# vwxyzjn/cleanrl

Measured on NVIDIA B200. Metric: env steps/sec (SPS) PPO Breakout num_envs=1024, higher is better.
Workload: dtype bf16

## Files before the change

### cleanrl_b200/_lib.py

```python
from __future__ import annotations

import ctypes as C
from pathlib import Path

PKG = Path(__file__).resolve().parent
LIB_PATH = PKG / "libb200rl.so"

_p = C.c_void_p
_i64 = C.c_int64
_i = C.c_int
_d = C.c_double
_sz = C.c_size_t

SIGNATURES = {
    "b200rl_version": (_i, []),
    "b200rl_last_error": (C.c_char_p, []),
    "b200rl_compiled_arch": (_i, []),
    "b200rl_launch_count": (C.c_longlong, []),
    "b200rl_profile_enable": (None, [_i]),
    "b200rl_profile_reset": (None, []),
    "b200rl_profile_summary": (_i, [C.c_char_p, _sz]),
    "b200rl_gae_f32": (_i, [_p, _p, _p, _p, _p, _p, _p, _i64, _i64, _d, _d, _i, _p]),
    "b200rl_categorical_sample_f32": (_i, [_p, _i64, _p, _p, _i64, _i64, _i, _p, _p, _p, _p, _p]),
    "b200rl_categorical_eval_f32": (_i, [_p, _i64, _p, _i64, _i, _p, _p, _p]),
    "b200rl_ppo_loss_workspace_bytes": (_sz, [_i64]),
    "b200rl_ppo_loss_f32": (_i, [_p, _i64, _p, _i64, _p, _p, _p, _p, _p, _p, _i64, _i, _d, _d, _d, _i, _i,
                                 _p, _i64, _p, _i64, _p, _p, _sz, _p]),
    "b200rl_gaussian_sample_f32": (_i, [_p, _i64, _p, _p, _p, _i64, _i64, _i, _p, _p, _p, _p, _p]),
    "b200rl_gaussian_eval_f32": (_i, [_p, _i64, _p, _p, _i64, _i, _p, _p, _p]),
    "b200rl_ppo_loss_gaussian_workspace_bytes": (_sz, [_i64]),
    "b200rl_ppo_loss_gaussian_f32": (_i, [_p, _i64, _p, _p, _i64, _p, _p, _p, _p, _p, _p, _i64, _i, _d, _d, _d, _i, _i,
                                          _p, _i64, _p, _p, _i64, _p, _p, _sz, _p]),
    "b200rl_clip_adam_workspace_bytes": (_sz, [_i64]),
    "b200rl_clip_adam_f32": (_i, [_p, _p, _p, _p, _i64, _i64, _d, _d, _d, _d, _d, _i, _p, _p, _sz, _p]),
    "b200rl_adam_step_scalars": (_i, [_i64, _d, _d, _d, _p]),
    "b200rl_clip_adam_dyn_f32": (_i, [_p, _p, _p, _p, _i64, _p, _d, _d, _d, _d, _i, _p, _p, _sz, _p]),
    "b200rl_conv2d_fwd_f32": (_i, [_p, _i, _p, _d, _p, _p, _p, _i64, _i, _i, _i, _i, _i, _i, _i, _i, _p]),
    "b200rl_conv2d_bwd_data_f32": (_i, [_p, _p, _p, _i, _p, _i64, _i, _i, _i, _i, _i, _i, _i, _p]),
    "b200rl_conv2d_bwd_weight_workspace_bytes": (_sz, [_i64, _i, _i, _i, _i, _i, _i, _i]),
    "b200rl_conv2d_bwd_weight_f32": (_i, [_p, _i, _p, _d, _p, _p, _p, _i64, _i, _i, _i, _i, _i, _i, _i, _p, _sz, _p]),
    "b200rl_conv2d_fwd_pad_f32": (_i, [_p, _i, _p, _d, _p, _p, _p, _i64, _i, _i, _i, _i, _i, _i, _i, _i, _i, _p]),
    "b200rl_conv2d_bwd_data_pad_f32": (_i, [_p, _p, _p, _i, _p, _i64, _i, _i, _i, _i, _i, _i, _i, _i, _p]),
    "b200rl_conv2d_bwd_weight_pad_workspace_bytes": (_sz, [_i64, _i, _i, _i, _i, _i, _i, _i, _i]),
    "b200rl_conv2d_bwd_weight_pad_f32": (_i, [_p, _i, _p, _d, _p, _p, _p, _i64, _i, _i, _i, _i, _i, _i, _i, _i, _p, _sz, _p]),
    "b200rl_maxpool3s2_fwd_f32": (_i, [_p, _i64, _i, _i, _p, _p, _p]),
    "b200rl_maxpool3s2_bwd_f32": (_i, [_p, _p, _i64, _i, _i, _p, _p]),
    "b200rl_relu_f32": (_i, [_p, _i64, _p, _p]),
    "b200rl_relu_bwd_f32": (_i, [_p, _p, _p, _i64, _p, _p]),
    "b200rl_add_f32": (_i, [_p, _p, _i64, _p, _p]),
    "b200rl_nhwc_to_nchw_u8": (_i, [_p, _p, _i64, _i, _i, _i, _p, _p]),
    "b200rl_linear_fwd_f32": (_i, [_p, _p, _p, _p, _p, _i64, _i, _i, _i, _p]),
    "b200rl_linear_bwd_data_f32": (_i, [_p, _p, _p, _i, _p, _i64, _i, _i, _p]),
    "b200rl_linear_bwd_weight_workspace_bytes": (_sz, [_i64, _i, _i]),
    "b200rl_linear_bwd_weight_f32": (_i, [_p, _p, _p, _p, _p, _i64, _i, _i, _p, _sz, _p]),
    "b200rl_dqn_td_loss_workspace_bytes": (_sz, [_i64]),
    "b200rl_dqn_td_loss_f32": (_i, [_p, _i64, _p, _i64, _p, _p, _p, _i64, _i, _d, _i, _p, _i64, _p, _p, _sz, _p]),
    "b200rl_argmax_f32": (_i, [_p, _i64, _i64, _i, _p, _p]),
    "b200rl_naturecnn_param_count": (_i64, [_i]),
    "b200rl_naturecnn_bf16_packed_bytes": (_sz, [_i]),
    "b200rl_naturecnn_bf16_acts_bytes": (_sz, [_i64, _i]),
    "b200rl_frames_to_s2d_bf16": (_i, [_p, _p, _i64, _p, _p]),
    "b200rl_naturecnn_bf16_workspace_bytes": (_sz, [_i64, _i]),
    "b200rl_naturecnn_bf16_pack": (_i, [_p, _i, _p, _p]),
    "b200rl_naturecnn_bf16_forward": (_i, [_p, _i, _p, _i64, _i, _p, _p, _p, _p, _p]),
    "b200rl_naturecnn_bf16_backward": (_i, [_p, _p, _i, _p, _i64, _i, _p, _p, _p, _p, _p, _p, _sz, _p, _p]),
    "b200rl_frames_to_s2d_u8": (_i, [_p, _p, _i64, _p, _p, _p]),
    "b200rl_lstm_mask_state_f32": (_i, [_p, _p, _p, _i64, _i, _p, _p, _p]),
    "b200rl_lstm_cell_fwd_f32": (_i, [_p, _p, _p, _i64, _i, _p, _p, _p, _p]),
    "b200rl_lstm_cell_bwd_f32": (_i, [_p, _p, _p, _p, _p, _p, _p, _i64, _i, _p, _p, _p]),
    "b200rl_naturecnn_grad_tail_offset": (_i64, [_i]),
    "b200rl_frames_delta_s2d_u8": (_i, [_p, _p, _p, _p, _p, _i64, _p, _p, _p]),
    "b200rl_h2d_rows_async": (_i, [_p, _p, _i64, _i64, _i64, _p]),
    "b200rl_stackdelta_create": (_p, [_i64, _i, _i64, _i]),
    "b200rl_stackdelta_destroy": (None, [_p]),
    "b200rl_stackdelta_invalidate": (None, [_p]),
    "b200rl_stackdelta_begin": (_i64, [_p, _p, _i64, _p, _p, _p, _p]),
    "b200rl_stackdelta_wait": (_i64, [_p, _p]),
    "b200rl_mt19937_shuffle_i64": (_i, [_p, _p, _p, _i64]),
    "b200rl_stackdelta_launch": (_i64, [_p, _p, _i64, _p]),
    "b200rl_stackdelta_join": (_i64, [_p, _p, _p]),
}



class PartLaunch(C.Structure):
    _fields_ = [("tracker", _p), ("copy_stream", _p), ("main_stream", _p), ("consumed_event", _p),
                ("n", C.c_int32), ("nchunks", C.c_int32), ("chunk_lo", C.c_int32 * 4), ("chunk_hi", C.c_int32 * 4),
                ("h2d_event", _p * 4), ("graph_exec", _p * 4),
                ("new_d", _p), ("slot_d", _p), ("full_d", _p), ("new_h", _p), ("full_h", _p), ("slot_h", _p),
                ("actions_d", _p), ("actions_h", _p), ("actions_bytes", _i64), ("d2h_event", _p)]


_lib = None


def load():
    global _lib
    if _lib is not None:
        return _lib
    if not LIB_PATH.exists():
        raise RuntimeError(
            f"{LIB_PATH} is missing: build it with `python -m cleanrl_b200.build` "
            "(the CUDA extension is the product; there is no CPU/torch fallback)")
    lib = C.CDLL(str(LIB_PATH))
    for name, (res, args) in SIGNATURES.items():
        fn = getattr(lib, name)
        fn.restype = res
        fn.argtypes = args
    _lib = lib
    return lib


def check(rc, what):
    if rc != 0:
        msg = load().b200rl_last_error().decode("utf-8", "replace")
        raise RuntimeError(f"libb200rl {what} failed (status {rc}): {msg}")
```

### cleanrl_b200/agents.py

```python
from __future__ import annotations

import numpy as np
import torch
import torch.nn as nn

from . import nets, ops


def layer_init(layer, std=np.sqrt(2), bias_const=0.0):
    torch.nn.init.orthogonal_(layer.weight, std)
    torch.nn.init.constant_(layer.bias, bias_const)
    return layer


def _exp_noise(n, A, device):
    return torch.empty(n, A, dtype=torch.float32, device=device).exponential_(1)


_exp_noise.graph_safe = True
_exp_noise.inplace = lambda buf: buf.exponential_(1)


class KernelAgent(nn.Module):

# ... 85 lines not shown
        return action, logprob, entropy, v.reshape(-1, 1)


class NatureCNNAgent(KernelAgent):

    def __init__(self, envs):
        super().__init__()
        c, h, w = envs.single_observation_space.shape
        assert (c, h, w) == (4, 84, 84), "NatureCNN geometry is 4x84x84"
        trunk = []
        for cin, cout, k, s in ((4, 32, 8, 4), (32, 64, 4, 2), (64, 64, 3, 1)):
            trunk += [layer_init(nn.Conv2d(cin, cout, k, stride=s)), nn.ReLU()]
        trunk += [nn.Flatten(), layer_init(nn.Linear(64 * 7 * 7, 512)), nn.ReLU()]
        self.network = nn.Sequential(*trunk)
        self.actor = layer_init(nn.Linear(512, envs.single_action_space.n), std=0.01)
        self.critic = layer_init(nn.Linear(512, 1), std=1)
        self.num_actions = int(envs.single_action_space.n)

    def _param_order(self):
        net = [p for m in self.network for p in m.parameters()]
        return net + [self.actor.weight, self.critic.weight, self.actor.bias, self.critic.bias]

    def _build_plan(self):
        f = self._flat
        A = self.num_actions
        wa, ga = f.view_of(self.actor.weight)
        ba, gba = f.view_of(self.actor.bias)
        off_w = (wa.data_ptr() - f.flat.data_ptr()) // 4
        off_b = (ba.data_ptr() - f.flat.data_ptr()) // 4
        self._head_w = f.flat[off_w:off_w + (A + 1) * 512].view(A + 1, 512)
        self._head_b = f.flat[off_b:off_b + A + 1]
        self._head_dw = f.grad[off_w:off_w + (A + 1) * 512].view(A + 1, 512)
        self._head_db = f.grad[off_b:off_b + A + 1]
        n = self.network
        self.trunk = nets.Chain([
            nets.Conv(n[0], "relu", in_div=255.0), nets.Conv(n[2], "relu"), nets.Conv(n[4], "relu"),
            nets.Linear(n[7], "relu")])
        self.head = nets.Linear(None, None, self._head_w, self._head_b, self._head_dw, self._head_db)
        self._tc = None
        self._tc_dirty = True

    precision = "fp32"

    def params_updated(self):
        self._tc_dirty = True

    def _tc_plan(self):
        f = self._flat
        if self._tc is None:
            assert f.flat.numel() >= ops._lib.load().b200rl_naturecnn_param_count(self.num_actions)
            self._tc = ops.NatureCNNBf16(self.num_actions, f.flat.device)
        if self._tc_dirty:
            self._tc.pack(f.flat)
            self._tc_dirty = False
        return self._tc

    def load_state_dict(self, *a, **k):
        out = super().load_state_dict(*a, **k)
        self._tc_dirty = True
        return out

    def pin_workspaces(self):
        if self._tc is not None:
            self._tc.pin()

    def _forward_heads(self, x, rows=None, keep=False, aux=None):
        if self.precision == "bf16":
            if x.dtype not in (torch.uint8, torch.bfloat16):
                x = x.to(torch.uint8)
            tc = self._tc_plan()
            out = tc.forward(x.contiguous(), rows, self._flat.flat)
            if keep:
                self._tc_obs, self._tc_rows, self._tc_aux = x, rows, aux
            A = self.num_actions
            return out[:, :A], out[:, A]
        if x.dtype not in (torch.uint8, torch.float32):
            x = x.float()
        hidden = self.trunk.fwd(x.contiguous(), rows=rows, keep=keep)
        out = self.head.fwd(hidden)
        if keep:
            self._hidden = hidden
        A = self.num_actions
        return out[:, :A], out[:, A]

    def forward_train(self, b_obs, mb_inds, aux=None):
        self.flat
        return self._forward_heads(b_obs, rows=mb_inds, keep=True, aux=aux)

    def alloc_head_grad(self, M, device):
        A = self.num_actions
        d = torch.empty(M, A + 1, dtype=torch.float32, device=device)
        return d, d[:, :A], d[:, A]

    def grad_tail(self):
        if self.precision != "bf16":
            return None
        if getattr(self, "_tail_event", None) is None:
            self._tail_event = torch.cuda.Event()
            self._tail_event.record()
        return self._tc_plan().grad_tail_offset(), self._tail_event

    def backward(self, dhead):
        if self.precision == "bf16":
            self._tc.backward(self._tc_obs, self._tc_rows, self._flat.flat, dhead, self._flat.grad,
                              tail_event=getattr(self, "_tail_event", None), obs_aux=getattr(self, "_tc_aux", None))
            self._tc_obs = self._tc_rows = self._tc_aux = None
            return
        hidden = self._hidden
        self.head.bwd_weight(hidden, dhead)
        dh = self.head.bwd_data(dhead, hidden, "relu")
        self.trunk.bwd(dh)
        self._hidden = None


class MLPAgent(KernelAgent):

    def __init__(self, envs):
        super().__init__()
        d = int(np.array(envs.single_observation_space.shape).prod())
        A = int(envs.single_action_space.n)
        self.critic = nn.Sequential(layer_init(nn.Linear(d, 64)), nn.Tanh(), layer_init(nn.Linear(64, 64)), nn.Tanh(),
                                    layer_init(nn.Linear(64, 1), std=1.0))
        self.actor = nn.Sequential(layer_init(nn.Linear(d, 64)), nn.Tanh(), layer_init(nn.Linear(64, 64)), nn.Tanh(),
                                   layer_init(nn.Linear(64, A), std=0.01))
        self.num_actions = A

    def _build_plan(self):
        mk = lambda seq: nets.Chain([nets.Linear(seq[0], "tanh"), nets.Linear(seq[2], "tanh"), nets.Linear(seq[4], None)])
        self.c_chain, self.a_chain = mk(self.critic), mk(self.actor)

    def _forward_heads(self, x, rows=None, keep=False):
        x = x.float() if x.dtype != torch.float32 else x
        x = x.reshape(x.shape[0], -1).contiguous()
        logits = self.a_chain.fwd(x, rows=rows, keep=keep)
        value = self.c_chain.fwd(x, rows=rows, keep=keep)
        return logits, value[:, 0]

    def forward_train(self, b_obs, mb_inds):
        self.flat
        return self._forward_heads(b_obs, rows=mb_inds, keep=True)

    def alloc_head_grad(self, M, device):
        dl = torch.empty(M, self.num_actions, dtype=torch.float32, device=device)
        dv = torch.empty(M, 1, dtype=torch.float32, device=device)
        return (dl, dv), dl, dv[:, 0]

    def backward(self, dhead):
        dl, dv = dhead
        self.a_chain.bwd(dl)
        self.c_chain.bwd(dv)


class LSTMAgent(KernelAgent):

    def __init__(self, envs):
        super().__init__()
        c, h, w = envs.single_observation_space.shape
        assert (h, w) == (84, 84), "NatureCNN trunk geometry is 84x84"
        trunk = []
        for cin, cout, k, s in ((c, 32, 8, 4), (32, 64, 4, 2), (64, 64, 3, 1)):
            trunk += [layer_init(nn.Conv2d(cin, cout, k, stride=s)), nn.ReLU()]
        trunk += [nn.Flatten(), layer_init(nn.Linear(64 * 7 * 7, 512)), nn.ReLU()]
        self.network = nn.Sequential(*trunk)
        self.lstm = nn.LSTM(512, 128)
        for name, param in self.lstm.named_parameters():
            if "bias" in name:
# ... 415 lines not shown
```

### cleanrl_b200/csrc/net_tc.cu

```cuda
#include <cuda.h>
#include "tc_base.cuh"
#include "tc_conv_win.cuh"
#include "tc_conv1_u8.cuh"
#include "tc_gemm_tma.cuh"
#include "tc_wgrad_win.cuh"
#include "tc_reduce.cuh"
#include "tc_aux.cuh"
#include "tc_heads.cuh"

namespace b200rl {

struct NatureLayout {
    int A;
    int64_t c1w, c1b, c2w, c2b, c3w, c3b, fcw, fcb, hw, hb, total;
    int64_t w1f, w2f, w2dg, w3f, w3dg, wfcf, wfcdg, w1l, w1sc, packed_total;
    explicit NatureLayout(int A_) : A(A_) {
        int64_t o = 0;
        c1w = o; o += 32 * 4 * 8 * 8;  c1b = o; o += 32;
        c2w = o; o += 64 * 32 * 4 * 4; c2b = o; o += 64;
        c3w = o; o += 64 * 64 * 3 * 3; c3b = o; o += 64;
        fcw = o; o += 512 * 3136;      fcb = o; o += 512;
        hw = o;  o += (int64_t)(A + 1) * 512;
        hb = o;  o += A + 1;
        total = o;
        int64_t q = 0;
        w1f = q; q += 32 * 256;
        w2f = q; q += 64 * 512;
        w2dg = q; q += 4 * 32 * 256;
        w3f = q; q += 64 * 576;
        w3dg = q; q += 64 * 576;
        wfcf = q; q += 512 * 3136;
        wfcdg = q; q += 3136 * 512;
        w1l = q; q += 64 * 256 / 2;
        w1sc = q; q += 64 * 2;
        packed_total = q;
    }
};

struct NatureActs {
    int64_t x0, act1, act2, act3, hid, dhid, dact3a, dact3b, dact2a, dact2b, dact1, m1, m2, m3, m4, total;
    explicit NatureActs(int64_t n, bool with_x0 = true) {
        int64_t o = 0;
        x0 = o; if (with_x0) o += n * 28224;
        act1 = o; o += n * 12800;
        act2 = o; o += n * 5184;
        act3 = o; o += n * 3136;
        hid = o;  o += n * 512;
        dhid = o; o += n * 512;
        dact3a = o; o += n * 5184;
        dact3b = o; o += n * 7744;
        dact2a = o; o += n * 6400;
        dact2b = o; o += n * 7744;
        dact1 = o; o += n * 14112;
        auto pad8 = [](int64_t v) { return (v + 7) & ~int64_t(7); };
        m1 = o; o += pad8(n * 100 * 4 * 2);
        m2 = o; o += pad8(n * 81 * 2 * 2);
        m3 = o; o += pad8(n * 49 * 2 * 2);
        m4 = o; o += pad8(n * 16 * 2);
        total = o;
    }
};

static void gemm_rowmajor(KGemmParams& p, const bf16* x, int64_t n, int nchunks) {
    memset(&p, 0, sizeof(p));
    p.scale = 1.f;
    p.A = x; p.M = n; p.nchunks = nchunks;
}


static void win_defaults(WinParams& p) { memset(&p, 0, sizeof(p)); p.scale = 1.f; }
static int round8(int v) { return (v + 7) & ~7; }
static void win_conv1(WinParams& p, const bf16* x0, const int64_t* rows, int64_t n) {
    p.A = x0; p.rows = rows; p.n = (int)n; p.G = 441; p.Wp = 21; p.M = n * 441;
    p.tpi_shift = 2;
    p.n_images = rows ? (int64_t)1 << 24 : n;
    p.ntaps = 4; p.shift[0] = 0; p.shift[1] = 1; p.shift[2] = 21; p.shift[3] = 22; p.WR = round8(128 + 22);
}
static void win_conv2(WinParams& p, const bf16* act1, int64_t n) {
    p.A = act1; p.n = (int)n; p.G = 100; p.Wp = 10; p.M = n * 100;
    p.ntaps = 4; p.shift[0] = 0; p.shift[1] = 1; p.shift[2] = 10; p.shift[3] = 11; p.WR = round8(128 + 11);
}
static void win_conv3(WinParams& p, const bf16* act2, int64_t n) {
    p.A = act2; p.n = (int)n; p.G = 81; p.Wp = 9; p.M = n * 81;
    p.ntaps = 9; for (int ky = 0; ky < 3; ++ky) for (int kx = 0; kx < 3; ++kx) p.shift[ky * 3 + kx] = ky * 9 + kx;
    p.WR = round8(128 + 20);
}
static void wgw_defaults(WGradWinParams& w) { memset(&w, 0, sizeof(w)); }

static int64_t round_up(int64_t a, int64_t b) { return ceil_div(a, b) * b; }

struct WPlan { int64_t rows_per_cta; int splits; };
// ... 88 lines not shown
    size_t b = 0;
    auto mb = [&](size_t v) { if (v > b) b = v; };
    mb(colsum_ws(n * 441, 32)); mb(colsum_ws(n * 100, 64)); mb(colsum_ws(n * 81, 64)); mb(colsum_ws(n, 512));
    mb((size_t)2 * ceil_div(n, heads_rows_per_block(n)) * (A + 1) * 514 * 4);
    return a + b + 512;
}

extern "C" int b200rl_naturecnn_bf16_pack(const float* params, int A, void* packed, void* stream) {
    B200RL_REQUIRE(params && packed && A >= 1 && A < kMaxHeads, "naturecnn_pack: bad arguments (A must be in [1,23])");
    B200RL_REQUIRE(aligned(packed, 16), "naturecnn_pack: packed buffer must be 16-B aligned");
    const NatureLayout L(A);
    bf16* P = reinterpret_cast<bf16*>(packed);
    cudaStream_t s = (cudaStream_t)stream;
    ProfScope ps(s, "pack_weights", 0, (double)L.total * 4 + (double)L.packed_total * 2);
    tc_pack_conv1_s2d<<<32, 256, 0, s>>>(params + L.c1w, P + L.w1f);
    tc_pack_conv1_i8<<<32, 256, 0, s>>>(params + L.c1w, reinterpret_cast<int8_t*>(P + L.w1l), reinterpret_cast<float*>(P + L.w1sc));
    tc_pack_conv2_cells<<<128, 256, 0, s>>>(params + L.c2w, P + L.w2f);
    tc_pack_conv_s2_classes<<<(unsigned)ceil_div(32768, 256), 256, 0, s>>>(params + L.c2w, 64, 32, P + L.w2dg);
    tc_pack_conv<<<(unsigned)ceil_div(36864, 256), 256, 0, s>>>(params + L.c3w, 64, 64, 3, 3, 0, P + L.w3f, P + L.w3dg);
    tc_pack_fc<<<dim3(512 / 8, 49 / 7), 256, 0, s>>>(params + L.fcw, 512, 49, P + L.wfcf, P + L.wfcdg);
    return check_launch("naturecnn_pack", 6);
}

extern "C" int b200rl_naturecnn_bf16_forward(const void* obs, int obs_format, const int64_t* rows, int64_t n, int A,
                                             const float* params, const void* packed, void* acts,
                                             float* head_out, void* stream) {
    B200RL_REQUIRE(n >= 0, "naturecnn_forward: negative n");
    if (n == 0) return B200RL_OK;
    B200RL_REQUIRE(obs && params && packed && acts && head_out, "naturecnn_forward: null pointer");
    B200RL_REQUIRE(A >= 1 && A < kMaxHeads, "naturecnn_forward: A=%d outside [1,23]", A);
    B200RL_REQUIRE(obs_format == B200RL_OBS_U8_NCHW || obs_format == B200RL_OBS_S2D_BF16 || obs_format == B200RL_OBS_S2D_U8,
                   "naturecnn_forward: bad obs_format %d", obs_format);
    B200RL_REQUIRE(aligned(obs, 16) && aligned(acts, 16) && aligned(packed, 16), "naturecnn_forward: misaligned buffer");
    B200RL_REQUIRE(n <= (int64_t)1 << 22, "naturecnn_forward: n too large");
    const NatureLayout L(A);
    const NatureActs Q(n, obs_format == B200RL_OBS_U8_NCHW);
    const bf16* P = reinterpret_cast<const bf16*>(packed);
    bf16* act = reinterpret_cast<bf16*>(acts);
    cudaStream_t s = (cudaStream_t)stream;
    int rc;
    KGemmParams p;
    WinParams wp;
    const bf16* x0 = reinterpret_cast<const bf16*>(obs);
    const int64_t* x0rows = rows;
    if (obs_format == B200RL_OBS_U8_NCHW) {
        if ((rc = b200rl_frames_to_s2d_bf16(reinterpret_cast<const uint8_t*>(obs), rows, n, act + Q.x0, stream))) return rc;
        x0 = act + Q.x0; x0rows = nullptr;
    }
    if (obs_format == B200RL_OBS_S2D_U8) {
        Conv1U8Params cp;
        memset(&cp, 0, sizeof(cp));
        cp.rows = rows; cp.n = (int)n; cp.n_images = rows ? (int64_t)1 << 24 : n;
        cp.limbs = reinterpret_cast<const int8_t*>(P + L.w1l); cp.sc = reinterpret_cast<const float*>(P + L.w1sc);
        cp.bias = params + L.c1b; cp.out = act + Q.act1; cp.mask_out = reinterpret_cast<uint32_t*>(act + Q.m1);
        ProfScope ps(s, "conv1_fwd", 2.0 * n * 400 * 32 * 256, (double)n * (28224 + 12800 * 2 + 1600));
        if ((rc = launch_conv1_i8(cp, obs, s, "naturecnn/conv1_i8"))) return rc;
    } else {
    win_defaults(wp); win_conv1(wp, x0, x0rows, n);
    wp.Bw = P + L.w1f; wp.N = 32; wp.vH = 20; wp.vW = 20; wp.out_mode = WOUT_S2D2; wp.out = act + Q.act1;
    wp.bias = params + L.c1b; wp.scale = 1.0f / 255.0f; wp.relu = 1; wp.mask_out = reinterpret_cast<uint32_t*>(act + Q.m1);
    { ProfScope ps(s, "conv1_fwd", 2.0 * n * 400 * 32 * 256, (double)n * ((28224 + 12800) * 2 + 1600));
      if ((rc = launch_conv_win<32, 1, 9, 4>(wp, s, "naturecnn/conv1"))) return rc; }
    }
    win_defaults(wp); win_conv2(wp, act + Q.act1, n);
    wp.Bw = P + L.w2f; wp.N = 64; wp.vH = 9; wp.vW = 9; wp.out_mode = WOUT_DENSE; wp.out = act + Q.act2;
    wp.bias = params + L.c2b; wp.relu = 1; wp.mask_out = reinterpret_cast<uint32_t*>(act + Q.m2);
    { ProfScope ps(s, "conv2_fwd", 2.0 * n * 81 * 64 * 512, (double)n * ((12800 + 5184) * 2 + 648));
      if ((rc = launch_conv_win<64, 2, 4, 4>(wp, s, "naturecnn/conv2"))) return rc; }
    win_defaults(wp); win_conv3(wp, act + Q.act2, n);
    wp.Bw = P + L.w3f; wp.N = 64; wp.vH = 7; wp.vW = 7; wp.out_mode = WOUT_DENSE; wp.out = act + Q.act3;
    wp.bias = params + L.c3b; wp.relu = 1; wp.mask_out = reinterpret_cast<uint32_t*>(act + Q.m3);
    { ProfScope ps(s, "conv3_fwd", 2.0 * n * 49 * 64 * 576, (double)n * ((5184 + 3136) * 2 + 392));
      if ((rc = launch_conv_win<64, 1, 6, 9>(wp, s, "naturecnn/conv3"))) return rc; }
    gemm_rowmajor(p, act + Q.act3, n, 49);
    p.Bw = P + L.wfcf; p.N = 512; p.out = act + Q.hid; p.ldo = 512; p.bias = params + L.fcb; p.relu = 1;
    p.mask_out = reinterpret_cast<uint32_t*>(act + Q.m4);
    { ProfScope ps(s, "fc_fwd", 2.0 * n * 512 * 3136, (double)n * (3136 + 512) * 2 + 512.0 * 3136 * 2);
      if (n <= 8192) { if ((rc = launch_gemm_tma<64, 8>(p, s, "naturecnn/fc"))) return rc; }
      else if ((rc = launch_gemm_tma<256, 4>(p, s, "naturecnn/fc"))) return rc; }
    { ProfScope ps(s, "heads_fwd", 2.0 * n * 512 * (A + 1), (double)n * (1024 + 4 * (A + 1)));
      int hb = (int)ceil_div(n, 8); if (hb > num_sms() * 8) hb = num_sms() * 8;
      tc_heads_fwd<<<hb, 256, (size_t)(A + 1) * 2048, s>>>(act + Q.hid, params + L.hw, params + L.hb, n, A + 1, 512, head_out); }
    return check_launch("naturecnn/heads");
}

extern "C" int b200rl_naturecnn_bf16_backward(const void* obs, const void* obs_aux, int obs_format, const int64_t* rows, int64_t n, int A,
                                              const float* params, const void* packed, void* acts,
                                              const float* dhead, float* grads,
                                              void* workspace, size_t workspace_bytes, void* tail_ready_event, void* stream) {
    B200RL_REQUIRE(n >= 1, "naturecnn_backward: n must be >= 1");
    B200RL_REQUIRE(obs && params && packed && acts && dhead && grads && workspace, "naturecnn_backward: null pointer");
    B200RL_REQUIRE(A >= 1 && A < kMaxHeads, "naturecnn_backward: A=%d outside [1,23]", A);
    B200RL_REQUIRE(aligned(workspace, 16), "naturecnn_backward: workspace misaligned");
    const size_t need = b200rl_naturecnn_bf16_workspace_bytes(n, A);
    if (workspace_bytes < need) return fail(B200RL_ERR_WORKSPACE, "naturecnn_backward: workspace %zu < %zu", workspace_bytes, need);
    B200RL_REQUIRE(obs_format == B200RL_OBS_U8_NCHW || obs_format == B200RL_OBS_S2D_BF16 || obs_format == B200RL_OBS_S2D_U8,
                   "naturecnn_backward: bad obs_format %d", obs_format);
    B200RL_REQUIRE(obs_format != B200RL_OBS_S2D_U8 || (obs_aux && aligned(obs_aux, 16)), "naturecnn_backward: the uint8 rollout needs obs_aux");
    const NatureLayout L(A);
    const NatureActs Q(n, obs_format == B200RL_OBS_U8_NCHW);
    const bf16* P = reinterpret_cast<const bf16*>(packed);
    bf16* act = reinterpret_cast<bf16*>(acts);
    cudaStream_t s = (cudaStream_t)stream;
    const bf16* x0 = obs_format == B200RL_OBS_U8_NCHW ? act + Q.x0 : reinterpret_cast<const bf16*>(obs);
    const int64_t* x0rows = obs_format == B200RL_OBS_U8_NCHW ? nullptr : rows;
    size_t big = 0;
    {
        auto mx = [&](size_t v) { if (v > big) big = v; };
        mx((size_t)wgrad_plan(n * 512, kC1Ctas, 128).splits * 256 * 64 * 4);
        mx((size_t)wgrad_plan(n * 100, kC2Ctas, 128).splits * 512 * 64 * 4);
        mx((size_t)wgrad_plan(n * 81, kC3Ctas, 128).splits * 640 * 64 * 4);
        mx((size_t)wgrad_plan(n, kFcSplits, 64).splits * 512 * (13 * 256) * 4);
        big = (big + 255) & ~(size_t)255;
    }
    float* wsbig = reinterpret_cast<float*>(workspace);
    float* wssmall = reinterpret_cast<float*>(reinterpret_cast<char*>(workspace) + big);
    int rc;
    const int A1 = A + 1;
    {
        const int64_t rpb = heads_rows_per_block(n);
        const int nb = (int)ceil_div(n, rpb);
        ProfScope ps(s, "heads_bwd", 4.0 * n * 512 * A1, (double)n * (2048 + 64 + 8 * A1));
        const size_t sd = (size_t)rpb * A1 * sizeof(float);
        if (A1 <= 8) tc_heads_bwd_weight<8><<<nb, 512, sd, s>>>(dhead, act + Q.hid, n, A1, 512, rpb, wssmall);
        else tc_heads_bwd_weight<kMaxHeads><<<nb, 512, sd, s>>>(dhead, act + Q.hid, n, A1, 512, rpb, wssmall);
        tc_heads_fold<<<(unsigned)ceil_div(A1 * 514, 32), 256, 0, s>>>(wssmall, 2 * nb, A1, 512, grads + L.hw, grads + L.hb);
        int db_blocks = (int)ceil_div(n * 64, 256); if (db_blocks > num_sms() * 8) db_blocks = num_sms() * 8;
        tc_heads_bwd_data<<<db_blocks, 256, (size_t)A1 * 2048, s>>>(dhead, params + L.hw, reinterpret_cast<const uint8_t*>(act + Q.m4), n, A1, 512, act + Q.dhid);
        if ((rc = check_launch("naturecnn/heads_bwd", 3))) return rc;
    }
    KGemmParams p;
    {
        const WPlan pl = wgrad_plan(n, kFcSplits, 64);
        { ProfScope ps(s, "fc_wgrad", 2.0 * n * 512 * 3136, (double)n * (3136 + 512) * 2 + 512.0 * 3136 * 4);
          CUtensorMap tmX, tmY;
          if ((rc = make_tmap_2d(&tmX, act + Q.dhid, n, 512, 64, "naturecnn/fc_wgrad"))) return rc;
          if ((rc = make_tmap_2d(&tmY, act + Q.act3, n, 3136, 64, "naturecnn/fc_wgrad"))) return rc;
          const size_t smem = (size_t)4 * (2 + 4) * 64 * 128 + 1024;
          static SmemAttrCache attr;
          if ((rc = attr.ensure(tc_wgrad_tma, smem, "naturecnn/fc_wgrad"))) return rc;
          tc_wgrad_tma<<<dim3(pl.splits, 4, 13), 160, smem, s>>>(tmX, tmY, n, pl.rows_per_cta, 2, 4, wsbig);
          if ((rc = check_launch("naturecnn/fc_wgrad"))) return rc; }
        { ProfScope ps(s, "wgrad_fold_bias", 0, 0);
          note_launches(1); tc_fold_fc<<<(unsigned)ceil_div((int64_t)512 * 3136, 256), 256, 0, s>>>(wsbig, pl.splits, 512, 13 * 256, 512, 3136, 64, 49, 1.f, grads + L.fcw);
          if ((rc = colsum(act + Q.dhid, n, 512, 512, wssmall, grads + L.fcb, s))) return rc; }
        if (tail_ready_event) {
            cudaError_t e = cudaEventRecord(reinterpret_cast<cudaEvent_t>(tail_ready_event), s);
            if (e != cudaSuccess) return fail(B200RL_ERR_CUDA, "naturecnn_backward: cudaEventRecord: %s", cudaGetErrorString(e));
        }
        gemm_rowmajor(p, act + Q.dhid, n, 8);
        p.Bw = P + L.wfcdg; p.N = 3136; p.out = act + Q.dact3a; p.out2 = act + Q.dact3b; p.dual_dact3 = 1;
        p.ldo = 3136; p.mask_bits = reinterpret_cast<const uint32_t*>(act + Q.m3);
        { ProfScope ps(s, "fc_dgrad", 2.0 * n * 512 * 3136, (double)n * ((3136 + 512) * 2 + 392) + 512.0 * 3136 * 2);
          if ((rc = launch_gemm_tma<256, 4>(p, s, "naturecnn/fc_dgrad"))) return rc; }
    }
    WGradWinParams gw;
    WinParams wp;
    FoldWin fw;
    {
        wgw_defaults(gw);
        gw.X = act + Q.act2; gw.M = n * 81; gw.n = (int)n; gw.G = 81; gw.cpr = 1; gw.nslots = 10; gw.WRX = round8(128 + 20);
        for (int t = 0; t < 9; ++t) gw.shift[t] = (t / 3) * 9 + (t % 3);
        const int st[10] = {0, 1, 2, 3, 4, 5, 6, 7, 7, 8};
        for (int k = 0; k < 10; ++k) { gw.slot_tap[k] = st[k]; gw.slot_cc[k] = 0; }
        gw.Y = act + Q.dact3a; gw.ldy = 64; gw.ncolsY = 64;
        const WPlan pl = wgrad_plan(n * 81, kC3Ctas, 128);
// ... 83 lines not shown
```

### cleanrl_b200/csrc/policy.cu

```cuda
#include "common.cuh"
#include <cfloat>

namespace b200rl {

constexpr int kMaxA = 64;

struct RowStats {
    float lse;
    float m2;
    float s2;
};

__device__ __forceinline__ RowStats row_stats(const float* __restrict__ x, int A) {
    float m = -INFINITY;
    for (int k = 0; k < A; ++k) m = fmaxf(m, x[k]);
    const float mm = (fabsf(m) == INFINITY) ? 0.f : m;
    float s = 0.f;
    for (int k = 0; k < A; ++k) s += expf(x[k] - mm);
    RowStats r;
    r.lse = logf(s) + mm;
    float m2 = -INFINITY;
    for (int k = 0; k < A; ++k) m2 = fmaxf(m2, x[k] - r.lse);
    float s2 = 0.f;
    for (int k = 0; k < A; ++k) s2 += expf((x[k] - r.lse) - m2);
    r.m2 = m2;
    r.s2 = s2;
    return r;
}

__global__ void __launch_bounds__(128) categorical_sample_kernel(
    const float* __restrict__ logits, int64_t ld, const float* __restrict__ noise,
    const float* __restrict__ value_in, int64_t ldv, int64_t n, int A,
    int64_t* __restrict__ action, float* __restrict__ logprob, float* __restrict__ entropy,
    float* __restrict__ value_out) {
    const int64_t i = (int64_t)blockIdx.x * blockDim.x + threadIdx.x;
    if (i >= n) return;
    const float* x = logits + i * ld;
    const float* q = noise + i * (int64_t)A;
    const RowStats rs = row_stats(x, A);
    float best = -INFINITY, ent = 0.f;
    int arg = 0;
    for (int k = 0; k < A; ++k) {
        const float nl = x[k] - rs.lse;
        const float p = expf(nl - rs.m2) / rs.s2;
        const float sc = p / q[k];
        if (sc > best) { best = sc; arg = k; }
        ent += fmaxf(nl, -FLT_MAX) * p;
    }
    action[i] = arg;
    logprob[i] = x[arg] - rs.lse;
    if (entropy) entropy[i] = -ent;
    if (value_out && value_in) value_out[i] = value_in[i * ldv];
}

__global__ void __launch_bounds__(128) categorical_eval_kernel(
    const float* __restrict__ logits, int64_t ld, const int64_t* __restrict__ action, int64_t n, int A,
    float* __restrict__ logprob, float* __restrict__ entropy) {
    const int64_t i = (int64_t)blockIdx.x * blockDim.x + threadIdx.x;
    if (i >= n) return;
    const float* x = logits + i * ld;
    const RowStats rs = row_stats(x, A);
    float ent = 0.f;
    for (int k = 0; k < A; ++k) {
        const float nl = x[k] - rs.lse;
        ent += fmaxf(nl, -FLT_MAX) * (expf(nl - rs.m2) / rs.s2);
    }
    int a = (int)action[i];
    a = a < 0 ? 0 : (a >= A ? A - 1 : a);
    logprob[i] = x[a] - rs.lse;
    if (entropy) entropy[i] = -ent;
}

__device__ __forceinline__ float adv_pass(const float* __restrict__ b_adv, const int64_t* __restrict__ inds, int64_t M,
                                          float mean, bool squared) {
    float s = 0.f;
    const int64_t step = blockDim.x;
    int64_t i = threadIdx.x;
    for (; i + 7 * step < M; i += 8 * step) {
        int64_t j[8];
        float v[8];
#pragma unroll
        for (int u = 0; u < 8; ++u) j[u] = inds ? __ldg(inds + i + u * step) : i + u * step;
#pragma unroll
        for (int u = 0; u < 8; ++u) v[u] = __ldg(b_adv + j[u]);
#pragma unroll
        for (int u = 0; u < 8; ++u) {
            const float d = v[u] - mean;
            s += squared ? d * d : v[u];
        }
    }
    for (; i < M; i += step) {
        const float v = b_adv[inds ? inds[i] : i];
        const float d = v - mean;
        s += squared ? d * d : v;
    }
    return s;
}
__global__ void __launch_bounds__(1024) adv_stats_kernel(
    const float* __restrict__ b_adv, const int64_t* __restrict__ inds, int64_t M, float* __restrict__ out2) {
    __shared__ float red[32];
    const float mean = block_sum(adv_pass(b_adv, inds, M, 0.f, false), red) / (float)M;
    const float ss = block_sum(adv_pass(b_adv, inds, M, mean, true), red);
    if (threadIdx.x == 0) {
        out2[0] = mean;
        out2[1] = sqrtf(ss / (float)(M - 1));
    }
}

constexpr int kLossThreads = 256;
constexpr int kNumStats = 7;

struct LossParams {
    const float* logits; int64_t ld;
    const float* value; int64_t ldv;
    const int64_t* inds;
    const int64_t* b_actions;
    const float* b_logprobs; const float* b_adv; const float* b_ret; const float* b_val;
    int64_t M; int A;
    float clip, ent_coef, vf_coef;
    int norm_adv, clip_vloss;
    float* dlogits; int64_t ldd;
    float* dvalue; int64_t lddv;
    float* stats;
    const float* adv_stats;
    float* partials;
    unsigned int* ticket;
};

__global__ void __launch_bounds__(kLossThreads) ppo_loss_kernel(LossParams P) {
    __shared__ float red[32];
    __shared__ bool is_last;
// ... 437 lines not shown
```

### cleanrl_b200/csrc/tc_base.cuh

```cuda
#pragma once
#include <cuda.h>
#include <cstring>
#include "common.cuh"
#include "tc_common.cuh"

namespace b200rl {
using namespace tc;
typedef __nv_bfloat16 bf16;

__device__ __forceinline__ int4 ldg16(const void* p) { return __ldg(reinterpret_cast<const int4*>(p)); }

typedef CUresult (*EncodeTiledFn)(CUtensorMap*, CUtensorMapDataType, cuuint32_t, void*, const cuuint64_t*, const cuuint64_t*,
                                  const cuuint32_t*, const cuuint32_t*, CUtensorMapInterleave, CUtensorMapSwizzle,
                                  CUtensorMapL2promotion, CUtensorMapFloatOOBfill);
static EncodeTiledFn g_encode = nullptr;
static int make_tmap_2d(CUtensorMap* tm, const void* base, int64_t rows, int64_t cols, int box_rows, const char* what) {
    if (!g_encode) {
        void* fn = nullptr;
        cudaDriverEntryPointQueryResult qres;
        cudaError_t e = cudaGetDriverEntryPoint("cuTensorMapEncodeTiled", &fn, cudaEnableDefault, &qres);
        if (e != cudaSuccess || qres != cudaDriverEntryPointSuccess || !fn)
            return fail(B200RL_ERR_CUDA, "%s: cuTensorMapEncodeTiled not available (%s)", what, cudaGetErrorString(e));
        g_encode = reinterpret_cast<EncodeTiledFn>(fn);
    }
    const cuuint64_t dims[2] = {(cuuint64_t)cols, (cuuint64_t)rows};
    const cuuint64_t strides[1] = {(cuuint64_t)cols * 2};
    const cuuint32_t box[2] = {64u, (cuuint32_t)box_rows};
    const cuuint32_t estr[2] = {1u, 1u};
    CUresult r = g_encode(tm, CU_TENSOR_MAP_DATA_TYPE_BFLOAT16, 2, const_cast<void*>(base), dims, strides, box, estr,
                          CU_TENSOR_MAP_INTERLEAVE_NONE, CU_TENSOR_MAP_SWIZZLE_128B, CU_TENSOR_MAP_L2_PROMOTION_L2_256B,
                          CU_TENSOR_MAP_FLOAT_OOB_FILL_NONE);
    if (r != CUDA_SUCCESS) return fail(B200RL_ERR_CUDA, "%s: cuTensorMapEncodeTiled failed (%d)", what, (int)r);
    return B200RL_OK;
}

static int make_tmap_3d(CUtensorMap* tm, const void* base, int64_t n_images, int64_t rows_per_image, int64_t cols, int box_rows,
                        const char* what) {
    if (!g_encode) {
        CUtensorMap dummy;
        int rc = make_tmap_2d(&dummy, base, 128, 64, 8, what);
        if (rc) return rc;
    }
    const cuuint64_t dims[3] = {(cuuint64_t)cols, (cuuint64_t)rows_per_image, (cuuint64_t)n_images};
    const cuuint64_t strides[2] = {(cuuint64_t)cols * 2, (cuuint64_t)rows_per_image * (cuuint64_t)cols * 2};
    const cuuint32_t box[3] = {64u, (cuuint32_t)box_rows, 1u};
    const cuuint32_t estr[3] = {1u, 1u, 1u};
    CUresult r = g_encode(tm, CU_TENSOR_MAP_DATA_TYPE_BFLOAT16, 3, const_cast<void*>(base), dims, strides, box, estr,
                          CU_TENSOR_MAP_INTERLEAVE_NONE, CU_TENSOR_MAP_SWIZZLE_128B, CU_TENSOR_MAP_L2_PROMOTION_L2_256B,
                          CU_TENSOR_MAP_FLOAT_OOB_FILL_NONE);
    if (r != CUDA_SUCCESS) return fail(B200RL_ERR_CUDA, "%s: cuTensorMapEncodeTiled (3-D) failed (%d)", what, (int)r);
    return B200RL_OK;
}

static int make_tmap_3d_u8(CUtensorMap* tm, const void* base, int64_t n_images, int64_t rows_per_image, int64_t cols, int64_t pitch,
                           int box_rows, int box_cols, const char* what) {
    if (!g_encode) {
        CUtensorMap dummy;
        int rc = make_tmap_2d(&dummy, base, 128, 64, 8, what);
        if (rc) return rc;
    }
    const cuuint64_t dims[3] = {(cuuint64_t)cols, (cuuint64_t)rows_per_image, (cuuint64_t)n_images};
    const cuuint64_t strides[2] = {(cuuint64_t)pitch, (cuuint64_t)rows_per_image * (cuuint64_t)pitch};
    const cuuint32_t box[3] = {(cuuint32_t)box_cols, (cuuint32_t)box_rows, 1u};
    const cuuint32_t estr[3] = {1u, 1u, 1u};
    CUresult r = g_encode(tm, CU_TENSOR_MAP_DATA_TYPE_UINT8, 3, const_cast<void*>(base), dims, strides, box, estr,
                          CU_TENSOR_MAP_INTERLEAVE_NONE,
                          box_cols == 64 ? CU_TENSOR_MAP_SWIZZLE_64B : (box_cols == 128 ? CU_TENSOR_MAP_SWIZZLE_128B : CU_TENSOR_MAP_SWIZZLE_NONE),
                          CU_TENSOR_MAP_L2_PROMOTION_L2_256B, CU_TENSOR_MAP_FLOAT_OOB_FILL_NONE);
    if (r != CUDA_SUCCESS) return fail(B200RL_ERR_CUDA, "%s: cuTensorMapEncodeTiled (u8 3-D) failed (%d)", what, (int)r);
    return B200RL_OK;
}

static int make_tmap_pairs_u8(CUtensorMap* tm, const void* base, int64_t n_images, const char* what) {
    if (!g_encode) {
        CUtensorMap dummy;
        int rc = make_tmap_2d(&dummy, base, 128, 64, 8, what);
        if (rc) return rc;
    }
    const cuuint64_t dims[3] = {128u, 221u, (cuuint64_t)n_images};
    const cuuint64_t strides[2] = {128u, 28224u};
    const cuuint32_t box[3] = {128u, 144u, 1u};
    const cuuint32_t estr[3] = {1u, 1u, 1u};
    CUresult r = g_encode(tm, CU_TENSOR_MAP_DATA_TYPE_UINT8, 3, const_cast<void*>(base), dims, strides, box, estr,
                          CU_TENSOR_MAP_INTERLEAVE_NONE, CU_TENSOR_MAP_SWIZZLE_128B, CU_TENSOR_MAP_L2_PROMOTION_L2_256B,
                          CU_TENSOR_MAP_FLOAT_OOB_FILL_NONE);
    if (r != CUDA_SUCCESS) return fail(B200RL_ERR_CUDA, "%s: cuTensorMapEncodeTiled (u8 pair rows) failed (%d)", what, (int)r);
    return B200RL_OK;
}

struct SmemAttrCache {
    size_t v[64] = {};
    template <class F>
    int ensure(F* func, size_t smem, const char* what) {
        int dev = 0;
        cudaGetDevice(&dev);
        const bool cached = dev >= 0 && dev < 64;
        if (cached && smem <= v[dev]) return B200RL_OK;
        cudaError_t e = cudaFuncSetAttribute(func, cudaFuncAttributeMaxDynamicSharedMemorySize, (int)smem);
        if (e != cudaSuccess) return fail(B200RL_ERR_CUDA, "%s: smem attribute (%zu B): %s", what, smem, cudaGetErrorString(e));
        if (cached) v[dev] = smem;
        return B200RL_OK;
    }
};

static int g_num_sms = 0;
static int num_sms() {
    if (g_num_sms == 0) {
        int dev = 0;
        cudaGetDevice(&dev);
        if (cudaDeviceGetAttribute(&g_num_sms, cudaDevAttrMultiProcessorCount, dev) != cudaSuccess || g_num_sms <= 0) g_num_sms = 148;
    }
    return g_num_sms;
}

}
```

### cleanrl_b200/csrc/tc_conv1_u8.cuh

```cuda
#pragma once
#include "tc_base.cuh"
#include <cuda_fp16.h>
#include <cstdlib>
#include "tc_conv_win.cuh"

namespace b200rl {
using namespace tc;

__device__ __forceinline__ void umma_i8(uint32_t tmem_d, uint64_t adesc, uint64_t bdesc, uint32_t idesc, uint32_t accumulate) {
    asm volatile(
        "{\n\t.reg .pred p;\n\t"
        "setp.ne.b32 p, %4, 0;\n\t"
        "tcgen05.mma.cta_group::1.kind::i8 [%0], %1, %2, %3, p;\n\t}\n" ::"r"(tmem_d),
        "l"(adesc), "l"(bdesc), "r"(idesc), "r"(accumulate)
        : "memory");
}
__device__ __forceinline__ void umma_f16_ts(uint32_t tmem_d, uint32_t tmem_a, uint64_t bdesc, uint32_t idesc, uint32_t accumulate) {
    asm volatile(
        "{\n\t.reg .pred p;\n\t"
        "setp.ne.b32 p, %4, 0;\n\t"
        "tcgen05.mma.cta_group::1.kind::f16 [%0], [%1], %2, %3, p;\n\t}\n" ::"r"(tmem_d),
        "r"(tmem_a), "l"(bdesc), "r"(idesc), "r"(accumulate)
        : "memory");
}
// ... 26 lines not shown
    return (uint64_t)((smem_addr & 0x3FFFFu) >> 4) | (1ull << 16) | (32ull << 32) | kDescVersion | kDescSwizzle64;
}
__device__ __forceinline__ uint32_t img64_off(int r, int c) { return (uint32_t)(r * 64 + ((c ^ ((r >> 1) & 3)) << 4)); }
__host__ __device__ constexpr uint32_t make_idesc_i8(int M, int N) {
    return (2u << 4) | (0u << 7) | (1u << 10) | ((uint32_t)(N >> 3) << 17) | ((uint32_t)(M >> 4) << 24);
}
__host__ __device__ constexpr uint32_t make_idesc_f16ts(int M, int N, int b_bf16, int b_mn_major) {
    return (1u << 4) | (0u << 7) | ((uint32_t)b_bf16 << 10) | ((uint32_t)b_mn_major << 16) | ((uint32_t)(N >> 3) << 17) |
           ((uint32_t)(M >> 4) << 24);
}

__global__ void __launch_bounds__(256) tc_frames_to_s2d_u8(const uint8_t* __restrict__ obs, const int64_t* __restrict__ rows, int64_t n,
                                                           uint8_t* __restrict__ out_rm, uint8_t* __restrict__ out_cm) {
    __shared__ __align__(16) uint8_t plane[7056];
    const int64_t i = blockIdx.x >> 2;
    const int c = blockIdx.x & 3;
    const int64_t img = rows ? rows[i] : i;
    const int4* src = reinterpret_cast<const int4*>(obs + img * 28224 + c * 7056);
    for (int t = threadIdx.x; t < 441; t += 256) reinterpret_cast<int4*>(plane)[t] = __ldg(src + t);
    __syncthreads();
    for (int pos = threadIdx.x; pos < 441; pos += 256) {
        const int Y = pos / 21, X = pos - Y * 21;
        const uint8_t* p = plane + (Y * 4) * 84 + X * 4;
        int4 v;
        v.x = *reinterpret_cast<const int*>(p); v.y = *reinterpret_cast<const int*>(p + 84);
        v.z = *reinterpret_cast<const int*>(p + 168); v.w = *reinterpret_cast<const int*>(p + 252);
        *reinterpret_cast<int4*>(out_rm + (i * 441 + pos) * 64 + c * 16) = v;
    }
    for (int t = threadIdx.x; t < 16 * 112; t += 256) {
        const int ch = t / 112, q = t - ch * 112;
        const int sy = ch >> 2, sx = ch & 3;
        uint32_t w = 0;
#pragma unroll
        for (int e = 0; e < 4; ++e) {
            const int pos = q * 4 + e;
            if (pos < 441) {
                const int Y = pos / 21, X = pos - Y * 21;
                w |= (uint32_t)plane[(Y * 4 + sy) * 84 + X * 4 + sx] << (8 * e);
            }
        }
        *reinterpret_cast<uint32_t*>(out_cm + (i * 64 + c * 16 + ch) * 448 + q * 4) = w;
    }
}

__global__ void __launch_bounds__(256) tc_pack_conv1_i8(const float* __restrict__ w, int8_t* __restrict__ limbs, float* __restrict__ sc) {
    __shared__ float red[32];
    const int co = blockIdx.x, idx = threadIdx.x;
    const float v = w[co * 256 + idx];
    float m = fabsf(v);
#pragma unroll
    for (int o = 16; o > 0; o >>= 1) m = fmaxf(m, __shfl_xor_sync(0xffffffffu, m, o));
    if ((idx & 31) == 0) red[idx >> 5] = m;
    __syncthreads();
    float mx = red[0];
#pragma unroll
    for (int k = 1; k < 8; ++k) mx = fmaxf(mx, red[k]);
    const float s = mx > 0.f ? mx * (128.0f / 127.0f) : 1.0f;
    const float u = v / s * 128.0f;
    float l1 = rintf(u);
    l1 = fminf(fmaxf(l1, -127.f), 127.f);
    float l2 = rintf((u - l1) * 128.0f);
    l2 = fminf(fmaxf(l2, -127.f), 127.f);
    const int kx = idx & 7, ky = (idx >> 3) & 7, c = idx >> 6;
    const int a = ky >> 2, sy = ky & 3, b = kx >> 2, sx = kx & 3;
    const int k = (a * 2 + b) * 64 + c * 16 + sy * 4 + sx;
    limbs[co * 256 + k] = (int8_t)l1;
    limbs[(32 + co) * 256 + k] = (int8_t)l2;
    if (idx == 0) {
        sc[co] = s / 128.0f / 255.0f;
        sc[32 + co] = s / 16384.0f / 255.0f;
    }
}

struct Conv1U8Params {
    const int64_t* rows;
    int n;
    int64_t n_images;
    const int8_t* limbs;
    const float* sc;
    const float* bias;
    bf16* out;
    uint32_t* mask_out;
};

constexpr bool kConv1I8Direct256 = true;
template <int STAGES, int DBG>
__global__ void __launch_bounds__(kConvWinThreads, 1) tc_conv1_i8(const __grid_constant__ CUtensorMap tmA, const Conv1U8Params p, int total_tiles) {
    constexpr int BN = 64, WR = 144, NTAPS = 4;
    constexpr int STAGE_BYTES = WR * 128;
    constexpr int B_CHUNK = BN * 64;
    constexpr int NT = 4;
    constexpr uint32_t TMEM_COLS = 2 * NT * BN;
    extern __shared__ uint8_t smem_raw[];
    __shared__ uint64_t full_bar[STAGES], empty_bar[STAGES], tfull_bar[2 * NT], tempty_bar[2 * NT];
    __shared__ uint32_t tmem_base_smem;
    __shared__ __align__(16) float s_sc[32], s_bias[32];
    uint8_t* smem = reinterpret_cast<uint8_t*>((reinterpret_cast<uintptr_t>(smem_raw) + 1023) & ~uintptr_t(1023));
    const int tid = threadIdx.x, warp = tid >> 5;
    uint8_t* sW = smem;
    uint8_t* sRing = smem + NTAPS * B_CHUNK;
    uint8_t* sStage = sRing + (size_t)STAGES * STAGE_BYTES;

    if (tid == 0) {
        for (int s = 0; s < STAGES; ++s) { mbar_init(&full_bar[s], 1); mbar_init(&empty_bar[s], 1); }
        for (int a = 0; a < 2 * NT; ++a) { mbar_init(&tfull_bar[a], 1); mbar_init(&tempty_bar[a], 4); }
        fence_barrier_init();
        tma_prefetch_desc(&tmA);
    }
    if (warp == 1) tmem_alloc(&tmem_base_smem, TMEM_COLS);
    for (int idx = tid; idx < NTAPS * BN * 4; idx += blockDim.x) {
        const int c16 = idx & 3;
        const int t = (idx >> 2) & 3;
        const int r = idx >> 4;
        *reinterpret_cast<int4*>(sW + t * B_CHUNK + img64_off(r, c16)) = ldg16(p.limbs + r * 256 + t * 64 + c16 * 16);
    }
    if (tid < 32) { s_sc[tid] = p.sc[32 + tid]; s_bias[tid] = p.bias[tid]; }
    fence_proxy_async_smem();
    tc_fence_before_sync();
    __syncthreads();
    tc_fence_after_sync();
    const uint32_t tmem_d = tmem_base_smem;
    const int tile_begin = (int)(((int64_t)total_tiles * blockIdx.x) / gridDim.x);
    const int tile_end = (int)(((int64_t)total_tiles * (blockIdx.x + 1)) / gridDim.x);

    if (warp == 0) {
        if (tid == 0) {
            uint32_t q = 0;
            int z_next = 0;
            if (tile_begin < tile_end) {
                const int img = tile_begin >> 1;
                z_next = p.rows ? (int)__ldg(p.rows + img) : img;
            }
            for (int tile = tile_begin; tile < tile_end; ++tile, ++q) {
                const uint32_t s = q % STAGES;
                const int z = z_next;
                if (tile + 1 < tile_end) {
                    const int img = (tile + 1) >> 1;
                    z_next = p.rows ? (int)__ldg(p.rows + img) : img;
                }
                if (q >= (uint32_t)STAGES) mbar_wait(&empty_bar[s], ((q / STAGES) - 1) & 1);
                if (DBG & 2) { mbar_arrive(&full_bar[s]); continue; }
                mbar_arrive_expect_tx(&full_bar[s], (uint32_t)STAGE_BYTES);
                tma_load_3d(smem_u32(sRing + (size_t)s * STAGE_BYTES), &tmA, 0, (tile & 1) * 128, z, &full_bar[s]);
            }
        }
    } else if (warp == 1) {
        const bool leader = elect_one();
        constexpr uint32_t idesc = make_idesc_i8(128, BN);
        const uint64_t a_hi = desc_kmajor(0) & 0xFFFFFFFF00000000ull;
        const uint32_t a_flags = (uint32_t)(desc_kmajor(0) & 0xFFFFFFFFull);
        const uint64_t b_hi = desc_kmajor_sw64(0) & 0xFFFFFFFF00000000ull;
        const uint32_t b_flags = (uint32_t)(desc_kmajor_sw64(0) & 0xFFFFFFFFull);
        const uint32_t w_lo = ((smem_u32(sW) & 0x3FFFFu) >> 4) | b_flags;
        constexpr int off[4] = {0, 1, 21, 22};
        uint32_t q = 0;
        for (int tile = tile_begin; tile < tile_end; ++tile, ++q) {
            const uint32_t s = q % STAGES;
            mbar_wait(&full_bar[s], (q / STAGES) & 1);
            const uint32_t win_lo = ((smem_u32(sRing + (size_t)s * STAGE_BYTES) & 0x3FFFFu) >> 4) | a_flags;
#pragma unroll
            for (int e = 0; e < 2; ++e) {
                const uint32_t acc = 2 * (q % NT) + e;
                if (q >= (uint32_t)NT) mbar_wait(&tempty_bar[acc], ((q / NT) - 1) & 1);
                tc_fence_after_sync();
                if (leader) {
                    const uint32_t d_addr = tmem_d + acc * BN;
#pragma unroll
                    for (int t = 0; t < NTAPS; ++t) {
                        if (DBG & 4) break;
                        const int po = e + off[t];
                        const uint32_t a_lo = win_lo + (uint32_t)((po >> 1) * 8 + (po & 1) * 4);
                        const uint32_t b_lo = w_lo + (uint32_t)((t * B_CHUNK) >> 4);
#pragma unroll
                        for (int kk = 0; kk < 2; ++kk)
                            umma_i8(d_addr, a_hi | (uint64_t)(a_lo + 2 * kk), b_hi | (uint64_t)(b_lo + 2 * kk), idesc,
                                    (t | kk) != 0 ? 1u : 0u);
                    }
                    if (e == 1) umma_commit(&empty_bar[s]);
                    umma_commit(&tfull_bar[acc]);
                }
                __syncwarp();
            }
        }
    } else {
        const int ew = warp & 3;
        const int grp = (warp - 2) >> 2;
        const int e = grp & 1, tp = grp >> 1;
        const int lrow = ew * 32 + (tid & 31);
        const uint32_t lane_base = tmem_d + ((uint32_t)(ew * 32) << 16);
        for (int tile = tile_begin + tp; tile < tile_end; tile += 2) {
            const uint32_t k = (uint32_t)(tile - tile_begin);
            const uint32_t acc = 2 * (k % NT) + e;
            const uint32_t lane_addr = lane_base + acc * BN;
            const int i = tile >> 1;
            const int rem = 2 * (((tile & 1) << 7) + lrow) + e;
            const int Y = (rem * 3121) >> 16, X = rem - Y * 21;
            const bool valid = rem < 441 && Y < 20 && X < 20;
            const int64_t cell = ((int64_t)i * 10 + (Y >> 1)) * 10 + (X >> 1);
            const int cls = (Y & 1) * 2 + (X & 1);
            mbar_wait(&tfull_bar[acc], (k / NT) & 1);
            tc_fence_after_sync();
            uint32_t a1[32], a2[32];
            if (DBG & 8) {
#pragma unroll
                for (int c4 = 0; c4 < 32; ++c4) { a1[c4] = (uint32_t)(tile + c4); a2[c4] = (uint32_t)(lrow * c4); }
            } else {
                tmem_ld32(lane_addr, a1);
                tmem_ld32(lane_addr + 32, a2);
                tmem_ld_wait();
            }
            tc_fence_before_sync();
            __syncwarp();
            if ((tid & 31) == 0) mbar_arrive(&tempty_bar[acc]);
            uint32_t bits = 0u;
            uint32_t pk[16];
#pragma unroll
            for (int c4 = 0; c4 < 32; c4 += 4) {
                const float4 sc = *reinterpret_cast<const float4*>(s_sc + c4);
                const float4 bi = *reinterpret_cast<const float4*>(s_bias + c4);
                const float f0 = fmaf((float)((int)a1[c4] * 128 + (int)a2[c4]), sc.x, bi.x);
                const float f1 = fmaf((float)((int)a1[c4 + 1] * 128 + (int)a2[c4 + 1]), sc.y, bi.y);
                const float f2 = fmaf((float)((int)a1[c4 + 2] * 128 + (int)a2[c4 + 2]), sc.z, bi.z);
                const float f3 = fmaf((float)((int)a1[c4 + 3] * 128 + (int)a2[c4 + 3]), sc.w, bi.w);
                bits |= (f0 > 0.f ? 1u : 0u) << c4;
                bits |= (f1 > 0.f ? 1u : 0u) << (c4 + 1);
                bits |= (f2 > 0.f ? 1u : 0u) << (c4 + 2);
                bits |= (f3 > 0.f ? 1u : 0u) << (c4 + 3);
                pk[c4 >> 1] = pack_bf16x2_relu(f0, f1);
                pk[(c4 >> 1) + 1] = pack_bf16x2_relu(f2, f3);
            }
            if (valid && !(DBG & 1)) p.mask_out[cell * 4 + cls] = bits;
            if (kConv1I8Direct256) {
                if (valid && !(DBG & 1)) {
                    uint8_t* dst = reinterpret_cast<uint8_t*>(p.out) + (cell * 4 + cls) * 64;
                    st_global_256(dst, make_int4((int)pk[0], (int)pk[1], (int)pk[2], (int)pk[3]), make_int4((int)pk[4], (int)pk[5], (int)pk[6], (int)pk[7]));
                    st_global_256(dst + 32, make_int4((int)pk[8], (int)pk[9], (int)pk[10], (int)pk[11]),
                                  make_int4((int)pk[12], (int)pk[13], (int)pk[14], (int)pk[15]));
                }
                continue;
            }
            uint8_t* stg = sStage + (size_t)(warp - 2) * 2304;
            const int lane = tid & 31;
            {
                const uint32_t f = (uint32_t)(lane >> 1) & 3u;
#pragma unroll
                for (int c = 0; c < 4; ++c)
                    *reinterpret_cast<int4*>(stg + lane * 64 + ((((uint32_t)c) ^ f) << 4)) =
                        make_int4((int)pk[4 * c], (int)pk[4 * c + 1], (int)pk[4 * c + 2], (int)pk[4 * c + 3]);
                reinterpret_cast<int*>(stg + 2048)[lane] = valid ? (int)(cell * 4 + cls) : -1;
            }
            __syncwarp();
#pragma unroll
            for (int i2 = 0; i2 < 4; ++i2) {
                const int R = (lane >> 2) + 8 * i2, c = lane & 3;
                const int unit = reinterpret_cast<const int*>(stg + 2048)[R];
                const int4 v = *reinterpret_cast<const int4*>(stg + R * 64 + ((((uint32_t)c) ^ ((uint32_t)(R >> 1) & 3u)) << 4));
                if (unit >= 0 && !(DBG & 1)) *reinterpret_cast<int4*>(reinterpret_cast<uint8_t*>(p.out) + (int64_t)unit * 64 + c * 16) = v;
            }
            __syncwarp();
        }
    }
    tc_fence_before_sync();
    __syncthreads();
    if (warp == 1) tmem_dealloc(tmem_d, TMEM_COLS);
}

struct Conv1WgradU8Params {
    const int64_t* rows;
    int n;
    int64_t rows_per_cta;
    float* ws;
    float* wsb;
};
constexpr int kC1WXStages = 12, kC1WYStages = 14;
constexpr int kC1WBlock = 64 * 128, kC1WYBytes = 128 * 64, kC1WYPadRows = 24, kC1WYPad = kC1WYPadRows * 64;
constexpr int kC1WShift = 21;
constexpr float kDact1Scale = 4096.0f;

__device__ __forceinline__ uint32_t prmt(uint32_t a, uint32_t b, uint32_t sel) {
    uint32_t d;
    asm("prmt.b32 %0, %1, %2, %3;" : "=r"(d) : "r"(a), "r"(b), "r"(sel));
    return d;
}
template <int B, int NH>
__device__ __forceinline__ void u8_to_f16_biased(const uint32_t* W, uint32_t (&H)[NH]) {
#pragma unroll
    for (int j = 0; j < NH / 2; ++j) {
        uint32_t x = W[j];
        if (B == 1) x = prmt(W[j], W[j + 1], 0x4321u);
        if (B == 2) x = prmt(W[j], W[j + 1], 0x5432u);
        if (B == 3) x = prmt(W[j], W[j + 1], 0x6543u);
        H[2 * j] = prmt(x, 0x64646464u, 0x5140u);
        H[2 * j + 1] = prmt(x, 0x64646464u, 0x7362u);
    }
}
constexpr float kU8Bias = 1024.0f;

constexpr int kC1WConvWarps = 16;
constexpr int kC1WThreads = (4 + kC1WConvWarps + 4 + 2) * 32;
template <int DBG>
__global__ void __launch_bounds__(kC1WThreads, 1) tc_conv1_wgrad_u8(const __grid_constant__ CUtensorMap tmX, const __grid_constant__ CUtensorMap tmY,
                                                                  const __grid_constant__ CUtensorMap tmYpad, const Conv1WgradU8Params p) {
    constexpr int XS = kC1WXStages, YS = kC1WYStages;
    constexpr int NA = 6;
    constexpr uint32_t TMEM_COLS = 512, COL_D = 0, COL_A = 128;
    extern __shared__ uint8_t smem_raw[];
    __shared__ uint64_t xfull[XS], xempty[XS], yfull[YS], yempty[YS], a_full[NA], a_empty[NA], done_bar;
    __shared__ uint32_t tmem_base_smem;
    __shared__ float sRed[32 * 32], sBias[32];
    uint8_t* smem = reinterpret_cast<uint8_t*>((reinterpret_cast<uintptr_t>(smem_raw) + 1023) & ~uintptr_t(1023));
    uint8_t* sX = smem;
    uint8_t* sYpad = smem + (size_t)XS * kC1WBlock;
    uint8_t* sYb = sYpad + kC1WYPad;
// ... 267 lines not shown
```

### cleanrl_b200/csrc/tc_conv_win.cuh

```cuda
#pragma once
#include "tc_base.cuh"

namespace b200rl {
using namespace tc;

enum { WOUT_DENSE = 0, WOUT_S2D2 = 1, WOUT_DACT2 = 2, WOUT_DACT1 = 3 };
struct WinParams {
    const bf16* A;
    const int64_t* rows;
    int64_t M;
    int n, G, Wp;
    int tpi_shift;
    int64_t n_images;
    int ntaps;
    int shift[16];
    int WR;
    const bf16* Bw;
    int N;
    int vH, vW;
    int out_mode;
    bf16* out;
    bf16* out2;
    const uint32_t* mask_bits;
    uint32_t* mask_out;
    const float* bias;
    float scale;
    int relu;
    int out_f16;
};

__device__ __forceinline__ uint32_t pack_f16x2_sat(float lo, float hi) {
    uint32_t d;
    asm("cvt.rn.satfinite.f16x2.f32 %0, %1, %2;" : "=r"(d) : "f"(hi), "f"(lo));
    return d;
}

constexpr int kConvWinThreads = 576;
__host__ __device__ constexpr int conv_win_groups(int BN) { return BN >= 128 ? 2 : 4; }
__host__ __device__ constexpr int conv_win_threads(int BN) { return 64 + conv_win_groups(BN) * 128; }
__host__ __device__ constexpr int conv_win_acc_bufs(int BN) { return BN <= 128 ? 4 : 2; }
template <int BN, int CPR, int STAGES, int NTAPS>
__global__ void __launch_bounds__(conv_win_threads(BN), 1) tc_conv_win(const __grid_constant__ CUtensorMap tmA, const WinParams p,
                                                      int total_tiles) {
    constexpr int B_CHUNK = BN * 128;
    constexpr int NB = conv_win_acc_bufs(BN);
    constexpr int NG = conv_win_groups(BN);
    static_assert(NB % NG == 0, "every epilogue group owns NB / NG accumulator buffers");
    constexpr uint32_t TMEM_COLS = (NB * BN) < 32 ? 32 : NB * BN;
    extern __shared__ uint8_t smem_raw[];
    __shared__ uint64_t full_bar[STAGES], empty_bar[STAGES], tfull_bar[NB], tempty_bar[NB];
    __shared__ uint32_t tmem_base_smem;
    uint8_t* smem = reinterpret_cast<uint8_t*>((reinterpret_cast<uintptr_t>(smem_raw) + 1023) & ~uintptr_t(1023));
    const int tid = threadIdx.x, warp = tid >> 5;
    const int nchunks = p.ntaps * CPR;
    const int K = nchunks * 64;
    const int IMG = p.WR * 128;
    const int STAGE_BYTES = IMG * CPR;
    uint8_t* sW = smem;
    uint8_t* sRing = smem + (size_t)nchunks * B_CHUNK;

    if (tid == 0) {
        for (int s = 0; s < STAGES; ++s) { mbar_init(&full_bar[s], 1); mbar_init(&empty_bar[s], 1); }
        for (int a = 0; a < NB; ++a) { mbar_init(&tfull_bar[a], 1); mbar_init(&tempty_bar[a], 4); }
        fence_barrier_init();
        tma_prefetch_desc(&tmA);
    }
    if (warp == 1) tmem_alloc(&tmem_base_smem, TMEM_COLS);
    for (int idx = tid; idx < nchunks * BN * 8; idx += blockDim.x) {
        const int c16 = idx & 7;
        int t = idx >> 3;
        const int r = t % BN; const int j = t / BN;
        int4 v = make_int4(0, 0, 0, 0);
        if (r < p.N) v = ldg16(p.Bw + (int64_t)r * K + j * 64 + c16 * 8);
        *reinterpret_cast<int4*>(sW + (size_t)j * B_CHUNK + img_off(r, c16)) = v;
    }
    fence_proxy_async_smem();
    tc_fence_before_sync();
    __syncthreads();
    tc_fence_after_sync();
    const uint32_t tmem_d = tmem_base_smem;
    const int tile_begin = (int)(((int64_t)total_tiles * blockIdx.x) / gridDim.x);
    const int tile_end = (int)(((int64_t)total_tiles * (blockIdx.x + 1)) / gridDim.x);

    if (warp == 0) {
        if (tid == 0) {
            uint32_t q = 0;
            const int tmask = (1 << p.tpi_shift) - 1;
            int z_next = 0;
            if (p.tpi_shift && tile_begin < tile_end) {
                const int img = tile_begin >> p.tpi_shift;
                z_next = p.rows ? (int)__ldg(p.rows + img) : img;
            }
            for (int tile = tile_begin; tile < tile_end; ++tile, ++q) {
                const uint32_t s = q % STAGES;
                const int z = z_next;
                if (p.tpi_shift && tile + 1 < tile_end) {
                    const int img = (tile + 1) >> p.tpi_shift;
                    z_next = p.rows ? (int)__ldg(p.rows + img) : img;
                }
                if (q >= (uint32_t)STAGES) mbar_wait(&empty_bar[s], ((q / STAGES) - 1) & 1);
                const uint32_t dst = smem_u32(sRing + (size_t)s * STAGE_BYTES);
                mbar_arrive_expect_tx(&full_bar[s], (uint32_t)STAGE_BYTES);
                if (p.tpi_shift) {
#pragma unroll
                    for (int c = 0; c < CPR; ++c) tma_load_3d(dst + c * IMG, &tmA, c * 64, (tile & tmask) * 128, z, &full_bar[s]);
                } else {
#pragma unroll
                    for (int c = 0; c < CPR; ++c) tma_load_2d(dst + c * IMG, &tmA, c * 64, tile * 128, &full_bar[s]);
                }
            }
        }
    } else if (warp == 1) {
        const bool leader = elect_one();
        constexpr uint32_t idesc = make_idesc(128, BN, 0, 0);
        const uint64_t desc_hi = desc_kmajor(0) & 0xFFFFFFFF00000000ull;
        const uint32_t desc_lo_flags = (uint32_t)(desc_kmajor(0) & 0xFFFFFFFFull);
        const uint32_t w_lo = ((smem_u32(sW) & 0x3FFFFu) >> 4) | desc_lo_flags;
// ... 11 lines not shown
                    for (int c = 0; c < CPR; ++c) {
                        const uint32_t a_lo = win_lo + (uint32_t)((c * IMG) >> 4) + (uint32_t)p.shift[t] * 8u;
                        const uint32_t b_lo = w_lo + (uint32_t)(((t * CPR + c) * B_CHUNK) >> 4);
#pragma unroll
                        for (int kk = 0; kk < 4; ++kk)
                            umma_bf16(d_addr, desc_hi | (uint64_t)(a_lo + 2 * kk), desc_hi | (uint64_t)(b_lo + 2 * kk), idesc,
                                      (t | c | kk) != 0 ? 1u : 0u);
                    }
                }
                umma_commit(&empty_bar[s]);
                umma_commit(&tfull_bar[acc]);
            }
            __syncwarp();
        }
    } else {
        const int ew = warp & 3;
        const int h = (warp - 2) >> 2;
        const int lrow = ew * 32 + (tid & 31);
        const uint32_t mW = (65536u + (uint32_t)p.Wp - 1u) / (uint32_t)p.Wp;
        constexpr int TSTEP = NG * 128;
        const int step_i = TSTEP / p.G, step_rem = TSTEP % p.G;
        int64_t r = ((int64_t)tile_begin + h) * 128 + lrow;
        int i_lin = (int)(r / p.G);
        int rem_lin = (int)(r - (int64_t)i_lin * p.G);
        const int tmask = (1 << p.tpi_shift) - 1;
        const uint32_t lane_base = tmem_d + ((uint32_t)(ew * 32) << 16);
        constexpr int NW = BN / 32;
        uint32_t k = 0;
        for (int tile = tile_begin + h; tile < tile_end; tile += NG, ++k) {
            const uint32_t acc = (uint32_t)(tile - tile_begin) % NB;
            const uint32_t lane_addr = lane_base + acc * BN;
            int i = i_lin, rem = rem_lin;
            bool inside = r < p.M;
            if (p.tpi_shift) {
                i = tile >> p.tpi_shift;
                rem = ((tile & tmask) << 7) + lrow;
                inside = rem < p.G;
            }
            const int Y = (int)(((uint32_t)rem * mW) >> 16), X = rem - Y * p.Wp;
            const bool valid = inside && (Y < p.vH) && (X < p.vW);
            int64_t o1 = 0, o2 = 0, ob = 0;
            if (p.out_mode == WOUT_DENSE) {
                const int64_t orow = ((int64_t)i * p.vH + Y) * p.vW + X;
                o1 = orow * p.N; ob = orow * (p.N >> 5);
            } else if (p.out_mode == WOUT_S2D2) {
                const int64_t cell = ((int64_t)i * 10 + (Y >> 1)) * 10 + (X >> 1);
                const int cls = (Y & 1) * 2 + (X & 1);
                o1 = cell * 128 + cls * 32; ob = cell * 4 + cls;
            } else if (p.out_mode == WOUT_DACT2) {
                o1 = ((int64_t)i * 100 + Y * 10 + X) * 64;
                o2 = ((int64_t)i * 121 + (Y + 1) * 11 + (X + 1)) * 64;
                ob = ((int64_t)i * 81 + Y * 9 + X) * 2;
            } else {
                ob = ((int64_t)i * 100 + Y * 10 + X) * 4;
            }
            uint32_t mb[NW];
#pragma unroll
            for (int g = 0; g < NW; ++g) mb[g] = 0xFFFFFFFFu;
            if (p.mask_bits != nullptr && valid) {
                if (NW == 4) {
                    const int4 t = ldg16(p.mask_bits + ob);
                    mb[0] = (uint32_t)t.x; mb[1 % NW] = (uint32_t)t.y; mb[2 % NW] = (uint32_t)t.z; mb[3 % NW] = (uint32_t)t.w;
                } else if (NW == 2) {
                    const uint2 t = __ldg(reinterpret_cast<const uint2*>(p.mask_bits + ob));
                    mb[0] = t.x; mb[1 % NW] = t.y;
                } else {
                    mb[0] = __ldg(p.mask_bits + ob);
                }
            }
            mbar_wait(&tfull_bar[acc], ((uint32_t)(tile - tile_begin) / NB) & 1);
            tc_fence_after_sync();
#pragma unroll
            for (int g = 0; g < NW; ++g) {
                uint32_t v[32];
                tmem_ld32(lane_addr + g * 32, v);
                tmem_ld_wait();
                if (g == NW - 1) {
                    tc_fence_before_sync();
                    __syncwarp();
                    if ((tid & 31) == 0) mbar_arrive(&tempty_bar[acc]);
                }
                if (!valid || g * 32 >= p.N) continue;
                if (p.bias) {
                    const float4* bp = reinterpret_cast<const float4*>(p.bias + g * 32);
#pragma unroll
                    for (int e = 0; e < 8; ++e) {
                        const float4 bv = __ldg(bp + e);
                        v[4 * e] = __float_as_uint(fmaf(__uint_as_float(v[4 * e]), p.scale, bv.x));
                        v[4 * e + 1] = __float_as_uint(fmaf(__uint_as_float(v[4 * e + 1]), p.scale, bv.y));
                        v[4 * e + 2] = __float_as_uint(fmaf(__uint_as_float(v[4 * e + 2]), p.scale, bv.z));
                        v[4 * e + 3] = __float_as_uint(fmaf(__uint_as_float(v[4 * e + 3]), p.scale, bv.w));
                    }
                } else {
#pragma unroll
                    for (int e = 0; e < 32; ++e) v[e] = __float_as_uint(__uint_as_float(v[e]) * p.scale);
                }
                if (p.relu) {
                    uint32_t bits = 0u;
#pragma unroll
                    for (int e = 0; e < 32; ++e) {
                        const float f = __uint_as_float(v[e]);
                        bits |= (f > 0.f ? 1u : 0u) << e;
                    }
                    if (p.mask_out) p.mask_out[ob + g] = bits;
                }
                if (p.mask_bits) {
#pragma unroll
                    for (int e = 0; e < 32; ++e) if (!((mb[g] >> e) & 1u)) v[e] = 0u;
                }
                int4 w[4];
                if (p.out_f16) {
#pragma unroll
                    for (int e = 0; e < 4; ++e) {
                        w[e].x = (int)pack_f16x2_sat(__uint_as_float(v[8 * e]), __uint_as_float(v[8 * e + 1]));
                        w[e].y = (int)pack_f16x2_sat(__uint_as_float(v[8 * e + 2]), __uint_as_float(v[8 * e + 3]));
                        w[e].z = (int)pack_f16x2_sat(__uint_as_float(v[8 * e + 4]), __uint_as_float(v[8 * e + 5]));
                        w[e].w = (int)pack_f16x2_sat(__uint_as_float(v[8 * e + 6]), __uint_as_float(v[8 * e + 7]));
                    }
                } else if (p.relu) {
#pragma unroll
                    for (int e = 0; e < 4; ++e) {
                        w[e].x = (int)pack_bf16x2_relu(__uint_as_float(v[8 * e]), __uint_as_float(v[8 * e + 1]));
                        w[e].y = (int)pack_bf16x2_relu(__uint_as_float(v[8 * e + 2]), __uint_as_float(v[8 * e + 3]));
                        w[e].z = (int)pack_bf16x2_relu(__uint_as_float(v[8 * e + 4]), __uint_as_float(v[8 * e + 5]));
                        w[e].w = (int)pack_bf16x2_relu(__uint_as_float(v[8 * e + 6]), __uint_as_float(v[8 * e + 7]));
                    }
                } else {
#pragma unroll
                for (int e = 0; e < 4; ++e) {
                    w[e].x = (int)pack_bf16x2(__uint_as_float(v[8 * e]), __uint_as_float(v[8 * e + 1]));
                    w[e].y = (int)pack_bf16x2(__uint_as_float(v[8 * e + 2]), __uint_as_float(v[8 * e + 3]));
                    w[e].z = (int)pack_bf16x2(__uint_as_float(v[8 * e + 4]), __uint_as_float(v[8 * e + 5]));
                    w[e].w = (int)pack_bf16x2(__uint_as_float(v[8 * e + 6]), __uint_as_float(v[8 * e + 7]));
                }
                }
                bf16* dst;
                if (p.out_mode == WOUT_DACT1) {
                    dst = p.out + ((int64_t)i * 441 + (2 * Y + (g >> 1)) * 21 + 2 * X + (g & 1)) * 32;
                } else {
                    dst = p.out + o1 + g * 32;
                }
                st_global_256(dst, w[0], w[1]);
                st_global_256(dst + 16, w[2], w[3]);
                if (p.out_mode == WOUT_DACT2) {
                    bf16* dst2 = p.out2 + o2 + g * 32;
                    st_global_256(dst2, w[0], w[1]);
                    st_global_256(dst2 + 16, w[2], w[3]);
                }
            }
            r += TSTEP; i_lin += step_i; rem_lin += step_rem;
            if (rem_lin >= p.G) { rem_lin -= p.G; ++i_lin; }
        }
    }
    tc_fence_before_sync();
    __syncthreads();
    if (warp == 1) tmem_dealloc(tmem_d, TMEM_COLS);
}

template <int BN, int CPR, int STAGES, int NTAPS>
static int launch_conv_win(const WinParams& p, cudaStream_t s, const char* what) {
    if (p.ntaps != NTAPS) return fail(B200RL_ERR_INVALID_ARGUMENT, "%s: %d taps, kernel instance has %d", what, p.ntaps, NTAPS);
    const size_t smem = (size_t)p.ntaps * CPR * BN * 128 + (size_t)STAGES * p.WR * 128 * CPR + 1024;
    static SmemAttrCache attr;
    if (int rc = attr.ensure(tc_conv_win<BN, CPR, STAGES, NTAPS>, smem, what)) return rc;
    if ((int64_t)p.G * p.Wp >= 65536 || p.G < 1 || p.N % 32 != 0)
        return fail(B200RL_ERR_INVALID_ARGUMENT, "%s: grid %d x width %d outside the epilogue's multiply-shift range, or N %% 32 != 0", what, p.G, p.Wp);
    if (p.rows && !p.tpi_shift) return fail(B200RL_ERR_INVALID_ARGUMENT, "%s: the image gather needs image-aligned tiling", what);
    if (p.tpi_shift && (128 << p.tpi_shift) < p.G) return fail(B200RL_ERR_INVALID_ARGUMENT, "%s: tiles per image too small", what);
    const int total = p.tpi_shift ? (int)((int64_t)p.n << p.tpi_shift) : (int)ceil_div(p.M, 128);
    int grid = num_sms();
    if (grid > total) grid = total;
    CUtensorMap tmA;
    memset(&tmA, 0, sizeof(tmA));
    int rc;
    if (p.tpi_shift) rc = make_tmap_3d(&tmA, p.A, p.n_images, p.G, (int64_t)CPR * 64, p.WR, what);
    else rc = make_tmap_2d(&tmA, p.A, p.M, (int64_t)CPR * 64, p.WR, what);
    if (rc) return rc;
    tc_conv_win<BN, CPR, STAGES, NTAPS><<<grid, conv_win_threads(BN), smem, s>>>(tmA, p, total);
    return check_launch(what);
}

}
```

### cleanrl_b200/csrc/tc_heads.cuh

```cuda
#pragma once
#include "tc_base.cuh"
#include "tc_reduce.cuh"

namespace b200rl {
using namespace tc;

constexpr int kMaxHeads = 24;
constexpr int kHeadsPartialBlocks = 296;
static inline int64_t heads_rows_per_block(int64_t n) {
    int64_t rpb = (n + kHeadsPartialBlocks - 1) / kHeadsPartialBlocks;
    if (rpb < 16) rpb = 16;
    if (rpb > 256) rpb = 256;
    return rpb;
}

__global__ void __launch_bounds__(256) tc_heads_fwd(const bf16* __restrict__ hid, const float* __restrict__ Wh,
                                                    const float* __restrict__ bh, int64_t n, int A1, int H,
                                                    float* __restrict__ out) {
    extern __shared__ float sW[];
    for (int i = threadIdx.x; i < A1 * 512; i += blockDim.x) sW[i] = Wh[i];
    __syncthreads();
    const int lane = threadIdx.x & 31, wpb = blockDim.x >> 5;
    for (int64_t row = (int64_t)blockIdx.x * wpb + (threadIdx.x >> 5); row < n; row += (int64_t)gridDim.x * wpb) {
        float hv[16];
        const bf16* hp = hid + row * 512;
#pragma unroll
        for (int q = 0; q < 2; ++q) {
            const int4 v = ldg16(hp + q * 256 + lane * 8);
            const uint32_t w[4] = {(uint32_t)v.x, (uint32_t)v.y, (uint32_t)v.z, (uint32_t)v.w};
#pragma unroll
            for (int e = 0; e < 4; ++e) {
                hv[q * 8 + 2 * e] = __uint_as_float(w[e] << 16);
                hv[q * 8 + 2 * e + 1] = __uint_as_float(w[e] & 0xFFFF0000u);
            }
        }
        float mine = 0.f;
        for (int a = 0; a < A1; ++a) {
            float s = 0.f;
#pragma unroll
            for (int q = 0; q < 2; ++q) {
                const float4 w0 = *reinterpret_cast<const float4*>(sW + a * 512 + q * 256 + lane * 8);
                const float4 w1 = *reinterpret_cast<const float4*>(sW + a * 512 + q * 256 + lane * 8 + 4);
                s = fmaf(hv[q * 8 + 0], w0.x, s); s = fmaf(hv[q * 8 + 1], w0.y, s);
                s = fmaf(hv[q * 8 + 2], w0.z, s); s = fmaf(hv[q * 8 + 3], w0.w, s);
                s = fmaf(hv[q * 8 + 4], w1.x, s); s = fmaf(hv[q * 8 + 5], w1.y, s);
                s = fmaf(hv[q * 8 + 6], w1.z, s); s = fmaf(hv[q * 8 + 7], w1.w, s);
            }
            s = warp_sum(s);
            if (lane == a) mine = s + bh[a];
        }
        if (lane < A1) out[row * A1 + lane] = mine;
    }
}
__global__ void __launch_bounds__(256) tc_heads_bwd_data(const float* __restrict__ dhead, const float* __restrict__ Wh,
                                                         const uint8_t* __restrict__ hid_bits, int64_t n, int A1, int H,
                                                         bf16* __restrict__ dhid) {
    extern __shared__ float sWt[];
    for (int i = threadIdx.x; i < A1 * 512; i += blockDim.x) {
        const int a = i >> 9, h = i & 511;
        sWt[a * 512 + (h & 7) * 64 + (h >> 3)] = Wh[i];
    }
    __syncthreads();
    const int64_t total = n * 64;
    for (int64_t idx = (int64_t)blockIdx.x * blockDim.x + threadIdx.x; idx < total; idx += (int64_t)gridDim.x * blockDim.x) {
        const int64_t row = idx >> 6;
        const int g = (int)(idx & 63);
        const uint32_t m = hid_bits[idx];
        float o[8];
#pragma unroll
        for (int e = 0; e < 8; ++e) o[e] = 0.f;
        for (int a = 0; a < A1; ++a) {
            const float d = __ldg(dhead + row * A1 + a);
#pragma unroll
            for (int e = 0; e < 8; ++e) o[e] = fmaf(d, sWt[a * 512 + e * 64 + g], o[e]);
        }
#pragma unroll
        for (int e = 0; e < 8; ++e) if (!((m >> e) & 1u)) o[e] = 0.f;
        int4 w;
        w.x = (int)pack_bf16x2(o[0], o[1]); w.y = (int)pack_bf16x2(o[2], o[3]);
        w.z = (int)pack_bf16x2(o[4], o[5]); w.w = (int)pack_bf16x2(o[6], o[7]);
        *reinterpret_cast<int4*>(dhid + row * 512 + g * 8) = w;
    }
}
template <int MAXA>
__global__ void __launch_bounds__(512) tc_heads_bwd_weight(const float* __restrict__ dhead, const bf16* __restrict__ hid,
                                                           int64_t n, int A1, int H, int64_t rows_per_block,
                                                           float* __restrict__ part) {
    extern __shared__ float sD[];
    const int hp = threadIdx.x & 255, rl = threadIdx.x >> 8;
    const int64_t r0 = (int64_t)blockIdx.x * rows_per_block;
    int64_t r1 = r0 + rows_per_block;
    if (r1 > n) r1 = n;
    const int nrows = (int)(r1 > r0 ? r1 - r0 : 0);
    for (int i = threadIdx.x; i < nrows * A1; i += blockDim.x) sD[i] = dhead[r0 * A1 + i];
    __syncthreads();
    float acc0[MAXA], acc1[MAXA], bacc[MAXA];
#pragma unroll
    for (int a = 0; a < MAXA; ++a) { acc0[a] = 0.f; acc1[a] = 0.f; bacc[a] = 0.f; }
    const uint32_t* h2 = reinterpret_cast<const uint32_t*>(hid);
    int r = rl;
    for (; r + 14 < nrows; r += 16) {
        uint32_t hv[8];
#pragma unroll
        for (int u = 0; u < 8; ++u) hv[u] = __ldg(h2 + (r0 + r + 2 * u) * 256 + hp);
#pragma unroll
        for (int u = 0; u < 8; ++u) {
            const float x0 = __uint_as_float(hv[u] << 16), x1 = __uint_as_float(hv[u] & 0xFFFF0000u);
            const float* dr = sD + (r + 2 * u) * A1;
#pragma unroll
            for (int a = 0; a < MAXA; ++a) {
                if (a < A1) {
                    const float d = dr[a];
                    acc0[a] = fmaf(d, x0, acc0[a]); acc1[a] = fmaf(d, x1, acc1[a]); bacc[a] += d;
                }
            }
        }
    }
    for (; r < nrows; r += 2) {
        const uint32_t hv = __ldg(h2 + (r0 + r) * 256 + hp);
        const float x0 = __uint_as_float(hv << 16), x1 = __uint_as_float(hv & 0xFFFF0000u);
        const float* dr = sD + r * A1;
#pragma unroll
        for (int a = 0; a < MAXA; ++a) {
            if (a < A1) {
                const float d = dr[a];
                acc0[a] = fmaf(d, x0, acc0[a]); acc1[a] = fmaf(d, x1, acc1[a]); bacc[a] += d;
            }
        }
    }
    float* pb = part + ((int64_t)blockIdx.x * 2 + rl) * A1 * (H + 2);
#pragma unroll
    for (int a = 0; a < MAXA; ++a) {
        if (a < A1) {
            *reinterpret_cast<float2*>(pb + (int64_t)a * (H + 2) + 2 * hp) = make_float2(acc0[a], acc1[a]);
// ... 17 lines not shown
```

### cleanrl_b200/ops.py

```python
from __future__ import annotations

import torch

from . import _lib

STAT_NAMES = ("pg_loss", "v_loss", "entropy", "old_approx_kl", "approx_kl", "clipfrac", "loss",
              "adv_mean", "adv_std")


def _stream():
    return torch.cuda.current_stream().cuda_stream


def _ptr(t, dtype=None, name="tensor", allow_none=False):
    if t is None:
        if allow_none:
            return None
        raise ValueError(f"{name} is None")
    if not isinstance(t, torch.Tensor) or not t.is_cuda:
        raise RuntimeError(f"{name}: libb200rl kernels need a CUDA tensor (got {type(t).__name__} on "
                           f"{getattr(t, 'device', '?')}); there is no CPU fallback")
    if dtype is not None and t.dtype != dtype:
        raise TypeError(f"{name}: expected {dtype}, got {t.dtype}")
    return t.data_ptr()
# ... 361 lines not shown
    lib = _lib.load()
    n, H = c_masked.shape
    f = torch.float32
    for nm, t in (("gates_x", gates_x), ("gates_h", gates_h), ("c_masked", c_masked), ("h_out", h_out), ("c_out", c_out)):
        _contig(t, nm)
    assert gates_x.shape == (n, 4 * H) and gates_h.shape == (n, 4 * H)
    rc = lib.b200rl_lstm_cell_fwd_f32(_ptr(gates_x, f, "gates_x"), _ptr(gates_h, f, "gates_h"), _ptr(c_masked, f, "c_masked"), n, H,
                                      _ptr(h_out, f, "h_out"), _ptr(c_out, f, "c_out"), _ptr(save, f, "save", True), _stream())
    _lib.check(rc, "lstm_cell_fwd")


def lstm_cell_bwd(dh_heads, dh_rec_raw, done_next, dc_rec, save, c_masked, done, dgates, dc_rec_out):
    lib = _lib.load()
    n, H = c_masked.shape
    f = torch.float32
    for nm, t in (("dh_heads", dh_heads), ("save", save), ("c_masked", c_masked), ("done", done), ("dgates", dgates),
                  ("dc_rec_out", dc_rec_out)):
        _contig(t, nm)
    rc = lib.b200rl_lstm_cell_bwd_f32(_ptr(dh_heads, f, "dh_heads"), _ptr(dh_rec_raw, f, "dh_rec_raw", True),
                                      _ptr(done_next, f, "done_next", True), _ptr(dc_rec, f, "dc_rec", True), _ptr(save, f, "save"),
                                      _ptr(c_masked, f, "c_masked"), _ptr(done, f, "done"), n, H, _ptr(dgates, f, "dgates"),
                                      _ptr(dc_rec_out, f, "dc_rec_out"), _stream())
    _lib.check(rc, "lstm_cell_bwd")


class NatureCNNBf16:

    def __init__(self, A, device):
        lib = _lib.load()
        self.A, self.device = int(A), device
        self.param_count = lib.b200rl_naturecnn_param_count(self.A)
        self.packed = torch.empty(lib.b200rl_naturecnn_bf16_packed_bytes(self.A), dtype=torch.uint8, device=device)
        self._acts = {}
        self._pinned = set()
        self._ws = None

    MAX_UNPINNED = 4

    def pin(self):
        self._pinned.update(self._acts.keys())

    def acts(self, n, fmt):
        lib = _lib.load()
        key = (n, fmt)
        buf = self._acts.pop(key, None)
        if buf is None:
            unpinned = [k for k in self._acts if k not in self._pinned]
            while len(unpinned) >= self.MAX_UNPINNED:
                del self._acts[unpinned.pop(0)]
            buf = torch.zeros(lib.b200rl_naturecnn_bf16_acts_bytes(n, fmt), dtype=torch.uint8, device=self.device)
        self._acts[key] = buf
        return buf

    @staticmethod
    def obs_format(obs):
        if obs.dtype == torch.uint8 and obs.dim() >= 4 and tuple(obs.shape[-3:]) == (4, 84, 84):
            return 0
        if obs.dtype == torch.bfloat16 and tuple(obs.shape[-3:]) == (21, 21, 64):
            return 1
        if obs.dtype == torch.uint8 and tuple(obs.shape[-2:]) == (441, 64):
            return 2
        raise TypeError("tensor-core NatureCNN path consumes uint8 [*,4,84,84] frames, uint8 space-to-depth rollout rows "
                        f"[*,441,64] or space-to-depth bf16 [*,21,21,64] (got {obs.dtype} {tuple(obs.shape)})")

    def pack(self, flat_params):
        lib = _lib.load()
        rc = lib.b200rl_naturecnn_bf16_pack(_ptr(flat_params, torch.float32, "params"), self.A,
                                            self.packed.data_ptr(), _stream())
        _lib.check(rc, "naturecnn_bf16_pack")

    def forward(self, obs, rows, flat_params, head_out=None):
        lib = _lib.load()
        fmt = self.obs_format(obs)
        _contig(obs, "obs")
        n = rows.numel() if rows is not None else obs.shape[0]
        if head_out is None:
            head_out = torch.empty(n, self.A + 1, dtype=torch.float32, device=self.device)
        rc = lib.b200rl_naturecnn_bf16_forward(_ptr(obs, None, "obs"), fmt, _ptr(rows, torch.int64, "rows", True), n, self.A,
                                               _ptr(flat_params, torch.float32, "params"), self.packed.data_ptr(),
                                               self.acts(n, fmt).data_ptr(), _ptr(head_out, torch.float32, "head_out"), _stream())
        _lib.check(rc, "naturecnn_bf16_forward")
        return head_out

    def grad_tail_offset(self):
        return int(_lib.load().b200rl_naturecnn_grad_tail_offset(self.A))

    def backward(self, obs, rows, flat_params, dhead, flat_grads, tail_event=None, obs_aux=None):
        lib = _lib.load()
        fmt = self.obs_format(obs)
        if fmt == 2:
            if obs_aux is None or obs_aux.dtype != torch.uint8 or tuple(obs_aux.shape[-2:]) != (64, 448) or \
                    obs_aux.shape[0] != obs.shape[0]:
                raise ValueError("uint8 rollout rows need their channel-major copy [*,64,448] (obs_aux) for the backward pass")
            _contig(obs_aux, "obs_aux")
        n = dhead.shape[0]
        _contig(dhead, "dhead")
        nbytes = lib.b200rl_naturecnn_bf16_workspace_bytes(n, self.A)
        if self._ws is None or self._ws.numel() < nbytes:
            self._ws = torch.empty(nbytes, dtype=torch.uint8, device=self.device)
        rc = lib.b200rl_naturecnn_bf16_backward(_ptr(obs, None, "obs"), _ptr(obs_aux, None, "obs_aux", True), fmt,
                                                _ptr(rows, torch.int64, "rows", True), n, self.A,
                                                _ptr(flat_params, torch.float32, "params"), self.packed.data_ptr(),
                                                self.acts(n, fmt).data_ptr(), _ptr(dhead, torch.float32, "dhead"),
                                                _ptr(flat_grads, torch.float32, "grads"),
                                                self._ws.data_ptr(), self._ws.numel(),
                                                tail_event.cuda_event if tail_event is not None else None, _stream())
        _lib.check(rc, "naturecnn_bf16_backward")


def frames_to_s2d(obs_u8, out=None, rows=None):
    lib = _lib.load()
    _contig(obs_u8, "obs")
    n = rows.numel() if rows is not None else obs_u8.shape[0]
    if out is None:
        out = torch.empty(n, 21, 21, 64, dtype=torch.bfloat16, device=obs_u8.device)
    rc = lib.b200rl_frames_to_s2d_bf16(_ptr(obs_u8, torch.uint8, "obs"), _ptr(rows, torch.int64, "rows", True), n,
                                       _ptr(out, torch.bfloat16, "out"), _stream())
    _lib.check(rc, "frames_to_s2d")
    return out


def alloc_u8_rollout_rows(shape, device):
    n = 1
    for d in shape:
        n *= int(d)
    flat = torch.zeros(n + 256, dtype=torch.uint8, device=device)
    return flat[:n].view(*shape)


def frames_to_s2d_u8(obs_u8, out_rm=None, out_cm=None, rows=None):
    lib = _lib.load()
    _contig(obs_u8, "obs")
    n = rows.numel() if rows is not None else obs_u8.shape[0]
    if out_rm is None:
        out_rm = alloc_u8_rollout_rows((n, 441, 64), obs_u8.device)
    if out_cm is None:
        out_cm = torch.empty(n, 64, 448, dtype=torch.uint8, device=obs_u8.device)
    _contig(out_rm, "out_rm"); _contig(out_cm, "out_cm")
    assert out_rm.shape[0] == n and out_cm.shape[0] == n
    rc = lib.b200rl_frames_to_s2d_u8(_ptr(obs_u8, torch.uint8, "obs"), _ptr(rows, torch.int64, "rows", True), n,
                                     _ptr(out_rm, torch.uint8, "out_rm"), _ptr(out_cm, torch.uint8, "out_cm"), _stream())
    _lib.check(rc, "frames_to_s2d_u8")
    return out_rm, out_cm


def frames_delta_s2d_u8(new_planes, prev_rm, prev_cm, out_rm, out_cm, full_slot=None, full_frames=None):
    lib = _lib.load()
    n = new_planes.shape[0]
    for nm, t in (("new_planes", new_planes), ("prev_rm", prev_rm), ("prev_cm", prev_cm), ("out_rm", out_rm), ("out_cm", out_cm)):
        _contig(t, nm)
        assert t.shape[0] == n, nm
    if full_slot is not None:
        _contig(full_slot, "full_slot"); _contig(full_frames, "full_frames")
        assert full_slot.shape[0] == n
    rc = lib.b200rl_frames_delta_s2d_u8(_ptr(new_planes, torch.uint8, "new_planes"), _ptr(full_slot, torch.int32, "full_slot", True),
                                        _ptr(full_frames, torch.uint8, "full_frames", True), _ptr(prev_rm, torch.uint8, "prev_rm"),
                                        _ptr(prev_cm, torch.uint8, "prev_cm"), n, _ptr(out_rm, torch.uint8, "out_rm"),
                                        _ptr(out_cm, torch.uint8, "out_cm"), _stream())
    _lib.check(rc, "frames_delta_s2d_u8")


def h2d_rows_async(dst, src_ptr, src_pitch, row_bytes, rows, stream=None):
    lib = _lib.load()
    assert dst.is_contiguous() and dst.numel() * dst.element_size() >= rows * row_bytes
    rc = lib.b200rl_h2d_rows_async(dst.data_ptr(), src_ptr, src_pitch, row_bytes, rows,
                                   stream.cuda_stream if stream is not None else _stream())
# ... 165 lines not shown
```

### cleanrl_b200/ppo_engine.py

```python
from __future__ import annotations

import os
import time

import numpy as np
import torch

from . import ops

STAT_NAMES = ops.STAT_NAMES


def _torch_dtype(np_dtype):
    return torch.uint8 if np.dtype(np_dtype) == np.uint8 else torch.float32


def _pin(t):
    return t.pin_memory() if torch.cuda.is_available() else t


def _sync():
    if torch.cuda.is_available():
        torch.cuda.current_stream().synchronize()

# ... 50 lines not shown
        self.next_done = torch.zeros(N, dtype=f32, device=device)
        self.next_value = torch.zeros(N, dtype=f32, device=device)
        self.rewards_h = _pin(torch.zeros((T, N), dtype=f32))
        self.dones_h = _pin(torch.zeros((T, N), dtype=f32))
        self.next_done_h = _pin(torch.zeros(N, dtype=f32))
        self.actions_h = _pin(torch.zeros_like(self.actions[0], device="cpu"))
        self.obs_stage_h = _pin(torch.zeros((N,) + tuple(obs_shape), dtype=self.obs_dtype))
        E = int(args.update_epochs)
        self.b_inds_h = _pin(torch.zeros((E, self.B), dtype=torch.int64))
        self.b_inds = torch.zeros((E, self.B), dtype=torch.int64, device=device)
        n_upd = int(args.update_epochs) * self.num_minibatches
        self.stats = torch.zeros(max(n_upd, 1), 16, dtype=f32, device=device)
        self.stats_h = _pin(torch.zeros(max(n_upd, 1), 16, dtype=f32))
        self.grad_norm = torch.zeros(1, dtype=f32, device=device)
        self.update_graphs = os.environ.get("CLEANRL_B200_UPDATE_GRAPHS", "1") != "0"
        self.host_seconds = {"shuffle": 0.0, "update_enqueue": 0.0, "update_wait": 0.0}
        self._shuffle = (ops.numpy_global_shuffle if device.type == "cuda" and os.environ.get("CLEANRL_B200_NATIVE_SHUFFLE", "1") != "0"
                         else np.random.shuffle)
        self._upd_graphs, self._upd_kernels, self._upd_iters = {}, {}, 0
        self.hyper = torch.zeros(max(n_upd, 1), 2, dtype=f32, device=device)
        self.hyper_h = _pin(torch.zeros(max(n_upd, 1), 2, dtype=f32))
        self.flat = agent.flat
        if self.overlap_exchange and hasattr(agent, "grad_tail"):
            agent.grad_tail()
        if cuda_graphs is None:
            cuda_graphs = os.environ.get("CLEANRL_B200_CUDA_GRAPHS", "1") != "0"
        self.cuda_graphs = bool(cuda_graphs) and device.type == "cuda"
        chunks = int(os.environ.get("CLEANRL_B200_H2D_CHUNKS", "4"))
        self.h2d_chunks = chunks if (self.cuda_graphs and getattr(self, "s2d", False) and chunks > 1
                                     and N % chunks == 0 and N // chunks >= 128) else 1
        C = self.h2d_chunks
        if C == 4 and N % 16 == 0:
            sizes = [5 * N // 16, 5 * N // 16, 4 * N // 16, 2 * N // 16]
        else:
            sizes = [N // C] * C
        self.chunk_bounds = [(sum(sizes[:c]), sum(sizes[:c + 1])) for c in range(C)]
        self.noise_buf = None
        if self.h2d_chunks > 1:
            self.copy_stream = torch.cuda.Stream(device=device)
            self.chunk_events = [torch.cuda.Event() for _ in range(self.h2d_chunks)]
            self.noise_buf = torch.zeros(agent.noise_shape(N), dtype=f32, device=device)
        self._parts = None
        want_delta = os.environ.get("CLEANRL_B200_DELTA_UPLOAD")
        if want_delta is None:
            want_delta = "1" if int(os.environ.get("LOCAL_WORLD_SIZE", "1") or 1) <= 1 else "0"
        self.delta_upload = bool(getattr(self, "u8_rollout", False)) and want_delta != "0"
        self._delta_allowed = self.delta_upload
        self._delta = None
        self.delta_redos = 0
        self.delta_full_frames = 0
        self._graphs = {}
        self._graph_pool = None
        self._graph_kernels = {}
        self._graph_warm = set()
        self.graph_launches = 0
        self.h2d_bytes = 0
        self.d2h_bytes = 0
        self.kernel_launches = 0

    def _to_storage(self, src_u8, step, sl=slice(None)):
        dst = self.next_obs if step is None else self.obs[step]
        if self.u8_rollout:
            dst_t = self.next_obs_t if step is None else self.obs_t[step]
            ops.frames_to_s2d_u8(src_u8, dst[sl], dst_t[sl])
        else:
            ops.frames_to_s2d(src_u8, out=dst[sl])

    def _upload_obs(self, step, obs_np, convert=True):
        dst = self.next_obs if step is None else self.obs[step]
        src = torch.from_numpy(np.ascontiguousarray(obs_np))
        if src.dtype != self.obs_dtype:
            src = src.to(self.obs_dtype)
        if not src.is_pinned():
            self.obs_stage_h.copy_(src)
            src = self.obs_stage_h
        if self.s2d:
            self.obs_u8.copy_(src, non_blocking=True)
            if convert:
                self._to_storage(self.obs_u8, step)
        else:
            dst.copy_(src, non_blocking=True)
        self.h2d_bytes += src.numel() * src.element_size()

    def _step_device_work(self, step, noise=None):
        if self.s2d:
            self._to_storage(self.obs_u8, step)
        self.agent.sample_into(self.obs[step], self.actions[step], self.logprobs[step], self.values[step], noise=noise)

    def _chunk_device_work(self, step, c):
        sl = slice(*self.chunk_bounds[c])
        self._to_storage(self.obs_u8[sl], step, sl)
        self.agent.sample_into(self.obs[step][sl], self.actions[step][sl], self.logprobs[step][sl],
                               self.values[step][sl], noise=self.noise_buf[sl])

    def _run_step(self, step, chunk=None):
        if chunk is not None:
            work, key = (lambda: self._chunk_device_work(step, chunk)), (step, chunk)
            return self._run_graphed(work, key, warm_key=("c", chunk))
        if self._graphable() and not getattr(self.agent.noise_fn, "graph_safe", False):
            if self.noise_buf is None:
                self.noise_buf = torch.zeros(self.agent.noise_shape(self.N), dtype=torch.float32, device=self.device)
            self.agent.draw_noise_into(self.noise_buf)
            return self._run_graphed(lambda: self._step_device_work(step, noise=self.noise_buf), step, warm_key=("f", 0))
        return self._run_graphed(lambda: self._step_device_work(step), step, warm_key=("f", 0))

    def _graphable(self):
        return self.cuda_graphs and getattr(self.agent, "graph_capturable", getattr(self.agent, "graph_friendly", False))

    def _run_graphed(self, work, key, warm_key):
        if not self._graphable():
            return work()
        if hasattr(self.agent, "_tc_plan") and getattr(self.agent, "precision", "fp32") == "bf16":
            self.agent._tc_plan()
        g = self._graphs.get(key)
        if g is None:
            if warm_key not in self._graph_warm:
                rng = torch.cuda.get_rng_state(self.device)
                work()
                torch.cuda.current_stream().synchronize()
                torch.cuda.set_rng_state(rng, self.device)
                self._graph_warm.add(warm_key)
            from . import _lib
            l0 = _lib.load().b200rl_launch_count()
            g = torch.cuda.CUDAGraph()
            if self._graph_pool is None:
                self._graph_pool = torch.cuda.graph_pool_handle()
            with torch.cuda.graph(g, pool=self._graph_pool):
                work()
            self._graphs[key] = g
            if hasattr(self.agent, "pin_workspaces"):
                self.agent.pin_workspaces()
            self._graph_kernels[key] = _lib.load().b200rl_launch_count() - l0
        g.replay()
        self.graph_launches += self._graph_kernels[key]

    @torch.no_grad()
    def policy_step(self, step, next_obs_np, next_done_np):
        if self.h2d_chunks > 1 and self._graphable():
            self._pipelined_step(step, next_obs_np)
            self.dones_h[step].copy_(torch.as_tensor(np.asarray(next_done_np, dtype=np.float32)))
        else:
            self.dones_h[step].copy_(torch.as_tensor(np.asarray(next_done_np, dtype=np.float32)))
            self._upload_obs(step, next_obs_np, convert=False)
            self._run_step(step)
        self.actions_h.copy_(self.actions[step], non_blocking=True)
        self.d2h_bytes += self.actions_h.numel() * self.actions_h.element_size()
        _sync()
        return self.actions_h.numpy()

    def _pipelined_step(self, step, obs_np):
        src = torch.from_numpy(np.ascontiguousarray(obs_np))
        if not src.is_pinned():
            self.obs_stage_h.copy_(src)
            src = self.obs_stage_h
        C = self.h2d_chunks
        main = torch.cuda.current_stream()
        with torch.cuda.stream(self.copy_stream):
            for c, (lo, hi) in enumerate(self.chunk_bounds):
                self.obs_u8[lo:hi].copy_(src[lo:hi], non_blocking=True)
                self.chunk_events[c].record(self.copy_stream)
        self.h2d_bytes += src.numel()
        self.agent.draw_noise_into(self.noise_buf)
        for c in range(C):
            main.wait_event(self.chunk_events[c])
            self._run_step(step, chunk=c)

    @torch.no_grad()
    def policy_step_resident(self, step, obs_dev, done_dev=None):
        if self.s2d and obs_dev.dtype == torch.uint8:
            self.obs_u8.copy_(obs_dev)
        else:
            self.obs[step].copy_(obs_dev)
        self._run_step(step)

    @torch.no_grad()
    def rollout_resident(self, obs_pool):
        P = obs_pool.shape[0]

        def work():
            for step in range(self.T):
                src = obs_pool[step % P]
                if self.s2d and src.dtype == torch.uint8:
                    self._to_storage(src, step)
                else:
                    self.obs[step].copy_(src)
                self.agent.sample_into(self.obs[step], self.actions[step], self.logprobs[step], self.values[step])

        if not getattr(self.agent, "graph_friendly", False):
            return work()
        self._run_graphed(work, ("rollout", obs_pool.data_ptr(), P), warm_key="r")

    def _part_setup(self, P):
        if getattr(self, "_parts", None) is not None and len(self._parts) == P:
            return
        N = self.N
        assert N % P == 0, "num_envs must be divisible by the number of env groups"
        n = N // P
        self._parts = [(p * n, (p + 1) * n) for p in range(P)]
        C = 2 if (n % 2 == 0 and n // 2 >= 64 and self.s2d and self._graphable()) else 1
        want = os.environ.get("CLEANRL_B200_PART_CHUNKS")
        if want and self.s2d and self._graphable() and 1 <= int(want) <= 4 and n % int(want) == 0:
            C = int(want)
        self._part_chunks = [[(lo + c * (n // C), lo + (c + 1) * (n // C)) for c in range(C)] for lo, hi in self._parts]
        if getattr(self, "copy_stream", None) is None:
            self.copy_stream = torch.cuda.Stream(device=self.device)
        self._part_h2d = [[torch.cuda.Event() for _ in ch] for ch in self._part_chunks]
        self._part_d2h = [torch.cuda.Event() for _ in range(P)]
        if self.noise_buf is None:
            self.noise_buf = torch.zeros(self.agent.noise_shape(N), dtype=torch.float32, device=self.device)
        if not hasattr(self, "obs_u8"):
            self.obs_u8 = None
        self._noise_bufs = [self.noise_buf, torch.zeros_like(self.noise_buf)]
        self._noise_step = -1
        self._actions_np = self.actions_h.numpy()
        self._rewards_np, self._dones_np = self.rewards_h.numpy(), self.dones_h.numpy()
        self._dones_ptr = self.dones_h.data_ptr()
        self._part_d2h_bytes = n * self.actions_h.element_size() * max(1, self.act_dim)
        self._part_d2h_handles = [None] * P
        self._plans, self._plan_refs, self._plan_kernels, self._plan_stream = {}, {}, {}, None
        if self.device.type == "cuda":
            from . import _lib
            self._lib = _lib.load()
        self._delta = None
        if self._delta_allowed and self._graphable():
            u8 = torch.uint8
            self._delta = [dict(tr=ops.StackDeltaTracker(n), full_d=torch.zeros((n, 28224), dtype=u8, device=self.device),
                                last=None, boot_obs=None, consumed=torch.cuda.Event()) for _ in range(P)]
            self._new_d = torch.zeros((N, 7056), dtype=u8, device=self.device)
            self._slot_d = torch.zeros(N, dtype=torch.int32, device=self.device)
            self._mis_ptr = [d["tr"].mis_h.data_ptr() for d in self._delta]

    def _part_work(self, step, lo, hi):
        sl = slice(lo, hi)
        if self.s2d:
            self._to_storage(self.obs_u8[sl], step, sl)
        self.agent.sample_into(self.obs[step][sl], self.actions[step][sl], self.logprobs[step][sl], self.values[step][sl],
                               noise=self._noise_bufs[step & 1][sl])

    @torch.no_grad()
    def launch_part(self, step, part, obs_np, done_np):
        if self._delta is not None and self.delta_upload:
            return self._launch_part_delta(step, part, obs_np, done_np)
        lo, hi = self._parts[part]
        src = torch.from_numpy(np.ascontiguousarray(obs_np))
        if src.dtype != self.obs_dtype:
            src = src.to(self.obs_dtype)
        if not src.is_pinned():
            self.obs_stage_h[lo:hi].copy_(src)
            src = self.obs_stage_h[lo:hi]
        main = torch.cuda.current_stream()
        dst = self.obs_u8 if self.s2d else self.obs[step]
        with torch.cuda.stream(self.copy_stream):
            for c, (clo, chi) in enumerate(self._part_chunks[part]):
                dst[clo:chi].copy_(src[clo - lo:chi - lo], non_blocking=True)
                self._part_h2d[part][c].record(self.copy_stream)
        self.h2d_bytes += src.numel() * src.element_size()
        self.dones_h[step][lo:hi].copy_(torch.as_tensor(np.asarray(done_np, dtype=np.float32)))
        if part == 0:
            self._ensure_noise(step)
        for c, (clo, chi) in enumerate(self._part_chunks[part]):
            main.wait_event(self._part_h2d[part][c])
            self._run_graphed(lambda: self._part_work(step, clo, chi), ("part", step, part, c), warm_key=("p", part, c))
        self.actions_h[lo:hi].copy_(self.actions[step][lo:hi], non_blocking=True)
        self._part_d2h[part].record(main)
        self.d2h_bytes += (hi - lo) * self.actions_h.element_size() * max(1, self.act_dim)

    def wait_actions(self, part):
        lo, hi = self._parts[part]
        if self._delta is not None:
            h = self._part_d2h_handles[part]
            if h is None:
                self._part_d2h[part].synchronize()
            self._join_part(part, h)
        else:
            self._part_d2h[part].synchronize()
        return self._actions_np[lo:hi]

    def _ensure_noise(self, step):
        if self._noise_step != step:
            self.agent.draw_noise_into(self._noise_bufs[step & 1])
            self._noise_step = step

    def _slot_pair(self, step):
        return (self.next_obs, self.next_obs_t) if step == self.T else (self.obs[step], self.obs_t[step])

    def _part_work_delta(self, step, part, lo, hi, sample, reuse):
        sl = slice(lo, hi)
        dst_rm, dst_cm = self._slot_pair(step)
        if reuse:
            dst_rm[sl].copy_(self.next_obs[sl])
            dst_cm[sl].copy_(self.next_obs_t[sl])
        else:
            prev_rm, prev_cm = self._slot_pair(self.T if step == 0 else step - 1)
            ops.frames_delta_s2d_u8(self._new_d[sl], prev_rm[sl], prev_cm[sl], dst_rm[sl], dst_cm[sl],
                                    full_slot=self._slot_d[sl], full_frames=self._delta[part]["full_d"])
        if sample:
            self.agent.sample_into(dst_rm[sl], self.actions[step][sl], self.logprobs[step][sl], self.values[step][sl],
                                   noise=self._noise_bufs[step & 1][sl])

    @staticmethod
    def _host_pinned(arr):
        try:
            return bool(torch.from_numpy(arr).is_pinned())
        except Exception:
            return False

    def _launch_part_delta(self, step, part, obs_np, done_np, sample=True):
        d = self._delta[part]
        reuse = step == 0 and d["boot_obs"] is not None and d["boot_obs"] is obs_np
        d["boot_obs"] = obs_np if step == self.T else None
        plan = self._plans.get((step, part, reuse))
        if plan is None or self._plan_stream != torch.cuda.current_stream().cuda_stream:
            return self._launch_part_delta_capture(step, part, obs_np, done_np, sample, reuse)
        lo, hi = self._parts[part]
        n = hi - lo
        lib = self._lib
        obs, optr, ostride = None, None, 0
        if not reuse:
            obs = obs_np
            if type(obs) is not np.ndarray or obs.dtype != np.uint8 or obs.ndim != 4 or obs.strides[1:] != (7056, 84, 1):
                obs = np.ascontiguousarray(obs_np, dtype=np.uint8)
            optr, ostride = obs.__array_interface__["data"][0], obs.strides[0]
            if step == 0:
                lib.b200rl_stackdelta_invalidate(d["tr"]._h)
        if sample:
            np.copyto(self._dones_np[step, lo:hi], done_np, casting="unsafe")
            dptr = self._dones_ptr + (step * self.N + lo) * 4
            if part == 0:
                self._ensure_noise(step)
        else:
            dkeep = np.ascontiguousarray(done_np, dtype=np.float32)
            dptr = dkeep.__array_interface__["data"][0]
        k = lib.b200rl_stackdelta_launch(self._plan_refs[(step, part, reuse)], optr, ostride, dptr)
        if k < 0:
            from . import _lib
            _lib.check(int(k), "stackdelta_launch")
        self.graph_launches += self._plan_kernels[(step, part, reuse)]
        if reuse:
            d["last"] = None
        else:
            self.h2d_bytes += n * (7056 + 4) + k * 28224
            self.delta_full_frames += k
            d["last"] = (step, obs, k, sample)
        if sample:
            self.d2h_bytes += self._part_d2h_bytes

    def _make_plan(self, step, part, reuse, sample):
        import ctypes
        from . import _lib
        lo, hi = self._parts[part]
        d = self._delta[part]
        tr = d["tr"]
        chunks = self._part_chunks[part]
        keys = [("dpart", step, part, c, reuse) for c in range(len(chunks))]
        if any(k not in self._graphs for k in keys):
            return
        pl = _lib.PartLaunch()
        pl.tracker = None if reuse else tr._h
        pl.copy_stream = self.copy_stream.cuda_stream
        pl.main_stream = torch.cuda.current_stream().cuda_stream
        pl.consumed_event = d["consumed"].cuda_event
        pl.n, pl.nchunks = hi - lo, len(chunks)
        for c, (clo, chi) in enumerate(chunks):
            pl.chunk_lo[c], pl.chunk_hi[c] = clo - lo, chi - lo
            pl.h2d_event[c] = self._part_h2d[part][c].cuda_event
            pl.graph_exec[c] = self._graphs[keys[c]].raw_cuda_graph_exec()
        pl.new_d, pl.slot_d, pl.full_d = self._new_d[lo:hi].data_ptr(), self._slot_d[lo:hi].data_ptr(), d["full_d"].data_ptr()
        pl.new_h, pl.full_h, pl.slot_h = tr.new_h.data_ptr(), tr.full_h.data_ptr(), tr.slot_h.data_ptr()
        if sample:
            pl.actions_d, pl.actions_h = self.actions[step][lo:hi].data_ptr(), self.actions_h[lo:hi].data_ptr()
            pl.actions_bytes = self._part_d2h_bytes
            pl.d2h_event = self._part_d2h[part].cuda_event
        key = (step, part, reuse)
        self._plans[key] = pl
        self._plan_refs[key] = ctypes.byref(pl)
        self._plan_kernels[key] = sum(self._graph_kernels[k] for k in keys)
        self._plan_stream = torch.cuda.current_stream().cuda_stream
        self._part_d2h_handles[part] = self._part_d2h[part].cuda_event

    def _launch_part_delta_capture(self, step, part, obs_np, done_np, sample, reuse):
        lo, hi = self._parts[part]
# ... 297 lines not shown
```

### include/b200rl.h

```cpp
#ifndef B200RL_H
#define B200RL_H

#include <stddef.h>
#include <stdint.h>

#ifdef __cplusplus
extern "C" {
#endif

typedef enum {
    B200RL_OK = 0,
    B200RL_ERR_INVALID_ARGUMENT = -1,
    B200RL_ERR_CUDA = -2,
    B200RL_ERR_UNSUPPORTED = -3,
    B200RL_ERR_WORKSPACE = -4
} b200rl_status;

int b200rl_version(void);
const char* b200rl_last_error(void);
int b200rl_compiled_arch(void);

long long b200rl_launch_count(void);
void b200rl_profile_enable(int on);
void b200rl_profile_reset(void);
// ... 51 lines not shown
                             int64_t P, const float* step_scalars, double beta1, double beta2, double eps,
                             double max_norm, int world_size, float* norm_out,
                             void* workspace, size_t workspace_bytes, void* stream);

enum { B200RL_ACT_NONE = 0, B200RL_ACT_RELU = 1, B200RL_ACT_TANH = 2 };
enum { B200RL_DT_F32 = 0, B200RL_DT_U8 = 1 };

int b200rl_conv2d_fwd_f32(const void* x, int x_dtype, const int64_t* rows, double in_div,
                          const float* w, const float* b, float* y,
                          int64_t n, int Cin, int H, int W, int Cout, int KH, int KW, int stride,
                          int act, void* stream);
int b200rl_conv2d_fwd_pad_f32(const void* x, int x_dtype, const int64_t* rows, double in_div,
                              const float* w, const float* b, float* y,
                              int64_t n, int Cin, int H, int W, int Cout, int KH, int KW, int stride, int pad,
                              int act, void* stream);
int b200rl_conv2d_bwd_data_pad_f32(const float* dy, const float* w, const float* x_post, int prev_act, float* dx,
                                   int64_t n, int Cin, int H, int W, int Cout, int KH, int KW, int stride, int pad, void* stream);
size_t b200rl_conv2d_bwd_weight_pad_workspace_bytes(int64_t n, int Cin, int H, int W, int Cout, int KH, int KW, int stride, int pad);
int b200rl_conv2d_bwd_weight_pad_f32(const void* x, int x_dtype, const int64_t* rows, double in_div,
                                     const float* dy, float* dw, float* db,
                                     int64_t n, int Cin, int H, int W, int Cout, int KH, int KW, int stride, int pad,
                                     void* workspace, size_t workspace_bytes, void* stream);
int b200rl_maxpool3s2_fwd_f32(const float* x, int64_t nc, int H, int W, float* y, uint8_t* argmax, void* stream);
int b200rl_maxpool3s2_bwd_f32(const float* dy, const uint8_t* argmax, int64_t nc, int H, int W, float* dx, void* stream);
int b200rl_relu_f32(const float* x, int64_t n, float* y, void* stream);
int b200rl_relu_bwd_f32(const float* dy, const float* x, const float* extra, int64_t n, float* dx, void* stream);
int b200rl_add_f32(const float* a, const float* b, int64_t n, float* y, void* stream);
int b200rl_nhwc_to_nchw_u8(const uint8_t* x, const int64_t* rows, int64_t n, int H, int W, int C, uint8_t* y, void* stream);
int b200rl_conv2d_bwd_data_f32(const float* dy, const float* w, const float* x_post, int prev_act,
                               float* dx,
                               int64_t n, int Cin, int H, int W, int Cout, int KH, int KW, int stride,
                               void* stream);
size_t b200rl_conv2d_bwd_weight_workspace_bytes(int64_t n, int Cin, int H, int W, int Cout, int KH, int KW, int stride);
int b200rl_conv2d_bwd_weight_f32(const void* x, int x_dtype, const int64_t* rows, double in_div,
                                 const float* dy, float* dw, float* db,
                                 int64_t n, int Cin, int H, int W, int Cout, int KH, int KW, int stride,
                                 void* workspace, size_t workspace_bytes, void* stream);
int b200rl_linear_fwd_f32(const float* x, const int64_t* rows, const float* w, const float* b, float* y,
                          int64_t n, int in_features, int out_features, int act, void* stream);
int b200rl_linear_bwd_data_f32(const float* dy, const float* w, const float* x_post, int prev_act, float* dx,
                               int64_t n, int in_features, int out_features, void* stream);
size_t b200rl_linear_bwd_weight_workspace_bytes(int64_t n, int in_features, int out_features);
int b200rl_linear_bwd_weight_f32(const float* x, const int64_t* rows, const float* dy, float* dw, float* db,
                                 int64_t n, int in_features, int out_features,
                                 void* workspace, size_t workspace_bytes, void* stream);

enum { B200RL_OBS_U8_NCHW = 0, B200RL_OBS_S2D_BF16 = 1, B200RL_OBS_S2D_U8 = 2 };
int b200rl_frames_to_s2d_bf16(const uint8_t* obs, const int64_t* rows, int64_t n, void* out_s2d, void* stream);
int b200rl_frames_to_s2d_u8(const uint8_t* obs, const int64_t* rows, int64_t n, uint8_t* out_rm, uint8_t* out_cm, void* stream);
int b200rl_frames_delta_s2d_u8(const uint8_t* new_planes, const int32_t* full_slot, const uint8_t* full_frames,
                               const uint8_t* prev_rm, const uint8_t* prev_cm, int64_t n,
                               uint8_t* out_rm, uint8_t* out_cm, void* stream);
int b200rl_h2d_rows_async(void* dst, const void* src, int64_t src_pitch, int64_t row_bytes, int64_t rows, void* stream);
void* b200rl_stackdelta_create(int64_t n_envs, int planes, int64_t plane_bytes, int threads);
void b200rl_stackdelta_destroy(void* tracker);
void b200rl_stackdelta_invalidate(void* tracker);
int64_t b200rl_stackdelta_begin(void* tracker, const uint8_t* obs, int64_t env_stride, const float* done,
                                uint8_t* new_out, uint8_t* full_out, int32_t* slot_out);
int64_t b200rl_stackdelta_wait(void* tracker, int32_t* mismatch_out);
typedef struct B200rlPartLaunch {
    void* tracker;
    void* copy_stream;
    void* main_stream;
    void* consumed_event;
    int32_t n, nchunks;
    int32_t chunk_lo[4], chunk_hi[4];
    void* h2d_event[4];
    void* graph_exec[4];
    uint8_t* new_d; int32_t* slot_d; uint8_t* full_d;
    uint8_t* new_h; uint8_t* full_h; int32_t* slot_h;
    const void* actions_d; void* actions_h; int64_t actions_bytes; void* d2h_event;
} B200rlPartLaunch;
int b200rl_mt19937_shuffle_i64(uint32_t* key624, int32_t* pos, int64_t* data, int64_t n);
int64_t b200rl_stackdelta_launch(const B200rlPartLaunch* plan, const uint8_t* obs, int64_t env_stride, const float* done);
int64_t b200rl_stackdelta_join(void* tracker, void* d2h_event, int32_t* mismatch_out);
int64_t b200rl_naturecnn_param_count(int A);
size_t b200rl_naturecnn_bf16_packed_bytes(int A);
size_t b200rl_naturecnn_bf16_acts_bytes(int64_t n, int obs_format);
size_t b200rl_naturecnn_bf16_workspace_bytes(int64_t n, int A);
int b200rl_naturecnn_bf16_pack(const float* params, int A, void* packed, void* stream);
int b200rl_naturecnn_bf16_forward(const void* obs, int obs_format, const int64_t* rows, int64_t n, int A,
                                  const float* params, const void* packed, void* acts,
                                  float* head_out, void* stream);
int b200rl_naturecnn_bf16_backward(const void* obs, const void* obs_aux, int obs_format, const int64_t* rows, int64_t n, int A,
                                   const float* params, const void* packed, void* acts,
                                   const float* dhead, float* grads,
                                   void* workspace, size_t workspace_bytes, void* tail_ready_event, void* stream);
int64_t b200rl_naturecnn_grad_tail_offset(int A);

int b200rl_lstm_mask_state_f32(const float* h, const float* c, const float* done, int64_t n, int H,
                               float* h_masked, float* c_masked, void* stream);
int b200rl_lstm_cell_fwd_f32(const float* gates_x, const float* gates_h, const float* c_masked, int64_t n, int H,
                             float* h_out, float* c_out, float* save, void* stream);
int b200rl_lstm_cell_bwd_f32(const float* dh_heads, const float* dh_rec_raw, const float* done_next, const float* dc_rec,
                             const float* save, const float* c_masked, const float* done, int64_t n, int H,
                             float* dgates, float* dc_rec_out, void* stream);

size_t b200rl_dqn_td_loss_workspace_bytes(int64_t B);
int b200rl_dqn_td_loss_f32(const float* q, int64_t ld_q, const float* q_target_next, int64_t ld_qt,
                           const int64_t* actions, const float* rewards, const float* dones,
                           int64_t B, int A, double gamma, int huber,
                           float* dq, int64_t ld_dq, float* stats,
                           void* workspace, size_t workspace_bytes, void* stream);
int b200rl_argmax_f32(const float* q, int64_t ld_q, int64_t n, int A, int64_t* out, void* stream);

#ifdef __cplusplus
}
#endif
#endif
```

Before: 2.184 million.

## Fuse rollout frame staging, conv tower, and head sampling into one path

Adds a fused rollout step for the bf16 NatureCNN. A single persistent tower kernel stages raw frames into the row- and channel-major observation slots, then runs conv1 through conv3. The FC GEMM follows, and a new heads kernel does categorical sampling, logprob and value in the same pass. This removes the separate storage-conversion kernel, the split forward/sample launches and the intermediate logits round trip. Risks are a much more complex warp-specialized kernel and changed launch/occupancy behaviour for small chunk sizes.

New measurement: 2.311 million, median of 6. +5.8%, better.

```diff
diff --git a/cleanrl_b200/_lib.py b/cleanrl_b200/_lib.py
--- a/cleanrl_b200/_lib.py
+++ b/cleanrl_b200/_lib.py
@@ -63,6 +63,7 @@
     "b200rl_naturecnn_bf16_workspace_bytes": (_sz, [_i64, _i]),
     "b200rl_naturecnn_bf16_pack": (_i, [_p, _i, _p, _p]),
     "b200rl_naturecnn_bf16_forward": (_i, [_p, _i, _p, _i64, _i, _p, _p, _p, _p, _p]),
+    "b200rl_naturecnn_bf16_rollout_step": (_i, [_p, _p, _p, _i64, _i, _p, _p, _p, _p, _p, _p, _p, _p]),
     "b200rl_naturecnn_bf16_backward": (_i, [_p, _p, _i, _p, _i64, _i, _p, _p, _p, _p, _p, _p, _sz, _p, _p]),
     "b200rl_frames_to_s2d_u8": (_i, [_p, _p, _i64, _p, _p, _p]),
     "b200rl_lstm_mask_state_f32": (_i, [_p, _p, _p, _i64, _i, _p, _p, _p]),
diff --git a/cleanrl_b200/agents.py b/cleanrl_b200/agents.py
--- a/cleanrl_b200/agents.py
+++ b/cleanrl_b200/agents.py
@@ -191,6 +191,11 @@
             self._hidden = hidden
         A = self.num_actions
         return out[:, :A], out[:, A]
+
+    def rollout_step_into(self, frames, slot_rm, slot_cm, actions_out, logprobs_out, values_out, noise=None):
+        n, A = slot_rm.shape[0], self.num_actions
+        q = noise if noise is not None else self.noise_fn(n, A, slot_rm.device)
+        self._tc_plan().rollout_step(frames, slot_rm, slot_cm, self._flat.flat, q, actions_out, logprobs_out, values_out)
 
     def forward_train(self, b_obs, mb_inds, aux=None):
         self.flat
diff --git a/cleanrl_b200/csrc/categorical.cuh b/cleanrl_b200/csrc/categorical.cuh
--- /dev/null
+++ b/cleanrl_b200/csrc/categorical.cuh
@@ -0,0 +1,46 @@
+#pragma once
+#include <cuda_runtime.h>
+#include <cfloat>
+
+namespace b200rl {
+
+struct RowStats {
+    float lse;
+    float m2;
+    float s2;
+};
+
+__device__ __forceinline__ RowStats row_stats(const float* __restrict__ x, int A) {
+    float m = -INFINITY;
+    for (int k = 0; k < A; ++k) m = fmaxf(m, x[k]);
+    const float mm = (fabsf(m) == INFINITY) ? 0.f : m;
+    float s = 0.f;
+    for (int k = 0; k < A; ++k) s += expf(x[k] - mm);
+    RowStats r;
+    r.lse = logf(s) + mm;
+    float m2 = -INFINITY;
+    for (int k = 0; k < A; ++k) m2 = fmaxf(m2, x[k] - r.lse);
+    float s2 = 0.f;
+    for (int k = 0; k < A; ++k) s2 += expf((x[k] - r.lse) - m2);
+    r.m2 = m2;
+    r.s2 = s2;
+    return r;
+}
+
+template <bool ENT>
+__device__ __forceinline__ int categorical_draw(const float* __restrict__ x, const float* __restrict__ q, int A, const RowStats& rs,
+                                                float* ent_out) {
+    float best = -INFINITY, ent = 0.f;
+    int arg = 0;
+    for (int k = 0; k < A; ++k) {
+        const float nl = x[k] - rs.lse;
+        const float p = expf(nl - rs.m2) / rs.s2;
+        const float sc = p / q[k];
+        if (sc > best) { best = sc; arg = k; }
+        if (ENT) ent += fmaxf(nl, -FLT_MAX) * p;
+    }
+    if (ENT) *ent_out = ent;
+    return arg;
+}
+
+}
diff --git a/cleanrl_b200/csrc/net_tc.cu b/cleanrl_b200/csrc/net_tc.cu
--- a/cleanrl_b200/csrc/net_tc.cu
+++ b/cleanrl_b200/csrc/net_tc.cu
@@ -7,6 +7,7 @@
 #include "tc_reduce.cuh"
 #include "tc_aux.cuh"
 #include "tc_heads.cuh"
+#include "tc_rollout_tower.cuh"
 
 namespace b200rl {
 
@@ -261,6 +262,43 @@
       int hb = (int)ceil_div(n, 8); if (hb > num_sms() * 8) hb = num_sms() * 8;
       tc_heads_fwd<<<hb, 256, (size_t)(A + 1) * 2048, s>>>(act + Q.hid, params + L.hw, params + L.hb, n, A + 1, 512, head_out); }
     return check_launch("naturecnn/heads");
+}
+
+extern "C" int b200rl_naturecnn_bf16_rollout_step(const uint8_t* frames, uint8_t* slot_rm, uint8_t* slot_cm, int64_t n, int A,
+                                                  const float* params, const void* packed, void* acts, const float* noise,
+                                                  int64_t* action, float* logprob, float* value, void* stream) {
+    B200RL_REQUIRE(n >= 0, "naturecnn_rollout_step: negative n");
+    if (n == 0) return B200RL_OK;
+    B200RL_REQUIRE(slot_rm && params && packed && acts && noise && action && logprob && value, "naturecnn_rollout_step: null pointer");
+    B200RL_REQUIRE(!frames || slot_cm, "naturecnn_rollout_step: raw frames need the channel-major slot");
+    B200RL_REQUIRE(A >= 1 && A < kMaxHeads, "naturecnn_rollout_step: A=%d outside [1,23]", A);
+    B200RL_REQUIRE(aligned(slot_rm, 16) && aligned(acts, 16) && aligned(packed, 16) && (!frames || (aligned(frames, 16) && aligned(slot_cm, 16))),
+                   "naturecnn_rollout_step: misaligned buffer");
+    B200RL_REQUIRE(n <= (int64_t)1 << 22, "naturecnn_rollout_step: n too large");
+    const NatureLayout L(A);
+    const NatureActs Q(n, false);
+    const bf16* P = reinterpret_cast<const bf16*>(packed);
+    bf16* act = reinterpret_cast<bf16*>(acts);
+    cudaStream_t s = (cudaStream_t)stream;
+    int rc;
+    TowerParams tp;
+    memset(&tp, 0, sizeof(tp));
+    tp.frames = frames; tp.slot_rm = slot_rm; tp.slot_cm = slot_cm; tp.n = (int)n;
+    tp.limbs = reinterpret_cast<const int8_t*>(P + L.w1l); tp.sc = reinterpret_cast<const float*>(P + L.w1sc); tp.b1 = params + L.c1b;
+    tp.w2 = P + L.w2f; tp.b2 = params + L.c2b; tp.w3 = P + L.w3f; tp.b3 = params + L.c3b; tp.act3 = act + Q.act3;
+    { ProfScope ps(s, "rollout_tower", 2.0 * n * (400 * 32 * 256 + 81 * 64 * 512 + 49 * 64 * 576),
+                   (double)n * ((frames ? 28224 * 2 + 28672 : 28224) + 3136 * 2));
+      if ((rc = launch_rollout_tower(tp, s, "naturecnn/rollout_tower"))) return rc; }
+    KGemmParams p;
+    gemm_rowmajor(p, act + Q.act3, n, 49);
+    p.Bw = P + L.wfcf; p.N = 512; p.out = act + Q.hid; p.ldo = 512; p.bias = params + L.fcb; p.relu = 1;
+    { ProfScope ps(s, "fc_fwd", 2.0 * n * 512 * 3136, (double)n * (3136 + 512) * 2 + 512.0 * 3136 * 2);
+      if (n <= 8192) { if ((rc = launch_gemm_tma<64, 8>(p, s, "naturecnn/fc"))) return rc; }
+      else if ((rc = launch_gemm_tma<256, 4>(p, s, "naturecnn/fc"))) return rc; }
+    { ProfScope ps(s, "rollout_heads_sample", 2.0 * n * 512 * (A + 1), (double)n * (1024 + 4 * A + 20));
+      int hb = (int)ceil_div(n, 8); if (hb > num_sms() * 8) hb = num_sms() * 8;
+      tc_heads_sample<<<hb, 256, (size_t)(A + 1) * 2048, s>>>(act + Q.hid, params + L.hw, params + L.hb, n, A, noise, action, logprob, value); }
+    return check_launch("naturecnn/heads_sample");
 }
 
 extern "C" int b200rl_naturecnn_bf16_backward(const void* obs, const void* obs_aux, int obs_format, const int64_t* rows, int64_t n, int A,
diff --git a/cleanrl_b200/csrc/policy.cu b/cleanrl_b200/csrc/policy.cu
--- a/cleanrl_b200/csrc/policy.cu
+++ b/cleanrl_b200/csrc/policy.cu
@@ -1,32 +1,10 @@
 #include "common.cuh"
+#include "categorical.cuh"
 #include <cfloat>
 
 namespace b200rl {
 
 constexpr int kMaxA = 64;
-
-struct RowStats {
-    float lse;
-    float m2;
-    float s2;
-};
-
-__device__ __forceinline__ RowStats row_stats(const float* __restrict__ x, int A) {
-    float m = -INFINITY;
-    for (int k = 0; k < A; ++k) m = fmaxf(m, x[k]);
-    const float mm = (fabsf(m) == INFINITY) ? 0.f : m;
-    float s = 0.f;
-    for (int k = 0; k < A; ++k) s += expf(x[k] - mm);
-    RowStats r;
-    r.lse = logf(s) + mm;
-    float m2 = -INFINITY;
-    for (int k = 0; k < A; ++k) m2 = fmaxf(m2, x[k] - r.lse);
-    float s2 = 0.f;
-    for (int k = 0; k < A; ++k) s2 += expf((x[k] - r.lse) - m2);
-    r.m2 = m2;
-    r.s2 = s2;
-    return r;
-}
 
 __global__ void __launch_bounds__(128) categorical_sample_kernel(
     const float* __restrict__ logits, int64_t ld, const float* __restrict__ noise,
@@ -38,15 +16,8 @@
     const float* x = logits + i * ld;
     const float* q = noise + i * (int64_t)A;
     const RowStats rs = row_stats(x, A);
-    float best = -INFINITY, ent = 0.f;
-    int arg = 0;
-    for (int k = 0; k < A; ++k) {
-        const float nl = x[k] - rs.lse;
-        const float p = expf(nl - rs.m2) / rs.s2;
-        const float sc = p / q[k];
-        if (sc > best) { best = sc; arg = k; }
-        ent += fmaxf(nl, -FLT_MAX) * p;
-    }
+    float ent;
+    const int arg = categorical_draw<true>(x, q, A, rs, &ent);
     action[i] = arg;
     logprob[i] = x[arg] - rs.lse;
     if (entropy) entropy[i] = -ent;
diff --git a/cleanrl_b200/csrc/tc_base.cuh b/cleanrl_b200/csrc/tc_base.cuh
--- a/cleanrl_b200/csrc/tc_base.cuh
+++ b/cleanrl_b200/csrc/tc_base.cuh
@@ -71,7 +71,7 @@
     return B200RL_OK;
 }
 
-static int make_tmap_pairs_u8(CUtensorMap* tm, const void* base, int64_t n_images, const char* what) {
+static int make_tmap_pairs_u8(CUtensorMap* tm, const void* base, int64_t n_images, const char* what, int box_rows = 144) {
     if (!g_encode) {
         CUtensorMap dummy;
         int rc = make_tmap_2d(&dummy, base, 128, 64, 8, what);
@@ -79,7 +79,7 @@
     }
     const cuuint64_t dims[3] = {128u, 221u, (cuuint64_t)n_images};
     const cuuint64_t strides[2] = {128u, 28224u};
-    const cuuint32_t box[3] = {128u, 144u, 1u};
+    const cuuint32_t box[3] = {128u, (cuuint32_t)box_rows, 1u};
     const cuuint32_t estr[3] = {1u, 1u, 1u};
     CUresult r = g_encode(tm, CU_TENSOR_MAP_DATA_TYPE_UINT8, 3, const_cast<void*>(base), dims, strides, box, estr,
                           CU_TENSOR_MAP_INTERLEAVE_NONE, CU_TENSOR_MAP_SWIZZLE_128B, CU_TENSOR_MAP_L2_PROMOTION_L2_256B,
diff --git a/cleanrl_b200/csrc/tc_conv1_u8.cuh b/cleanrl_b200/csrc/tc_conv1_u8.cuh
--- a/cleanrl_b200/csrc/tc_conv1_u8.cuh
+++ b/cleanrl_b200/csrc/tc_conv1_u8.cuh
@@ -132,6 +132,27 @@
     bf16* out;
     uint32_t* mask_out;
 };
+
+__device__ __forceinline__ uint32_t conv1_i8_epilogue(const uint32_t (&a1)[32], const uint32_t (&a2)[32], const float* s_sc,
+                                                      const float* s_bias, uint32_t (&pk)[16]) {
+    uint32_t bits = 0u;
+#pragma unroll
+    for (int c4 = 0; c4 < 32; c4 += 4) {
+        const float4 sc = *reinterpret_cast<const float4*>(s_sc + c4);
+        const float4 bi = *reinterpret_cast<const float4*>(s_bias + c4);
+        const float f0 = fmaf((float)((int)a1[c4] * 128 + (int)a2[c4]), sc.x, bi.x);
+        const float f1 = fmaf((float)((int)a1[c4 + 1] * 128 + (int)a2[c4 + 1]), sc.y, bi.y);
+        const float f2 = fmaf((float)((int)a1[c4 + 2] * 128 + (int)a2[c4 + 2]), sc.z, bi.z);
+        const float f3 = fmaf((float)((int)a1[c4 + 3] * 128 + (int)a2[c4 + 3]), sc.w, bi.w);
+        bits |= (f0 > 0.f ? 1u : 0u) << c4;
+        bits |= (f1 > 0.f ? 1u : 0u) << (c4 + 1);
+        bits |= (f2 > 0.f ? 1u : 0u) << (c4 + 2);
+        bits |= (f3 > 0.f ? 1u : 0u) << (c4 + 3);
+        pk[c4 >> 1] = pack_bf16x2_relu(f0, f1);
+        pk[(c4 >> 1) + 1] = pack_bf16x2_relu(f2, f3);
+    }
+    return bits;
+}
 
 constexpr bool kConv1I8Direct256 = true;
 template <int STAGES, int DBG>
@@ -262,23 +283,8 @@
             tc_fence_before_sync();
             __syncwarp();
             if ((tid & 31) == 0) mbar_arrive(&tempty_bar[acc]);
-            uint32_t bits = 0u;
             uint32_t pk[16];
-#pragma unroll
-            for (int c4 = 0; c4 < 32; c4 += 4) {
-                const float4 sc = *reinterpret_cast<const float4*>(s_sc + c4);
-                const float4 bi = *reinterpret_cast<const float4*>(s_bias + c4);
-                const float f0 = fmaf((float)((int)a1[c4] * 128 + (int)a2[c4]), sc.x, bi.x);
-                const float f1 = fmaf((float)((int)a1[c4 + 1] * 128 + (int)a2[c4 + 1]), sc.y, bi.y);
-                const float f2 = fmaf((float)((int)a1[c4 + 2] * 128 + (int)a2[c4 + 2]), sc.z, bi.z);
-                const float f3 = fmaf((float)((int)a1[c4 + 3] * 128 + (int)a2[c4 + 3]), sc.w, bi.w);
-                bits |= (f0 > 0.f ? 1u : 0u) << c4;
-                bits |= (f1 > 0.f ? 1u : 0u) << (c4 + 1);
-                bits |= (f2 > 0.f ? 1u : 0u) << (c4 + 2);
-                bits |= (f3 > 0.f ? 1u : 0u) << (c4 + 3);
-                pk[c4 >> 1] = pack_bf16x2_relu(f0, f1);
-                pk[(c4 >> 1) + 1] = pack_bf16x2_relu(f2, f3);
-            }
+            const uint32_t bits = conv1_i8_epilogue(a1, a2, s_sc, s_bias, pk);
             if (valid && !(DBG & 1)) p.mask_out[cell * 4 + cls] = bits;
             if (kConv1I8Direct256) {
                 if (valid && !(DBG & 1)) {
diff --git a/cleanrl_b200/csrc/tc_conv_win.cuh b/cleanrl_b200/csrc/tc_conv_win.cuh
--- a/cleanrl_b200/csrc/tc_conv_win.cuh
+++ b/cleanrl_b200/csrc/tc_conv_win.cuh
@@ -33,6 +33,27 @@
     uint32_t d;
     asm("cvt.rn.satfinite.f16x2.f32 %0, %1, %2;" : "=r"(d) : "f"(hi), "f"(lo));
     return d;
+}
+
+__device__ __forceinline__ void win_scale_bias32(uint32_t (&v)[32], const float* bias, float scale) {
+    const float4* bp = reinterpret_cast<const float4*>(bias);
+#pragma unroll
+    for (int e = 0; e < 8; ++e) {
+        const float4 bv = __ldg(bp + e);
+        v[4 * e] = __float_as_uint(fmaf(__uint_as_float(v[4 * e]), scale, bv.x));
+        v[4 * e + 1] = __float_as_uint(fmaf(__uint_as_float(v[4 * e + 1]), scale, bv.y));
+        v[4 * e + 2] = __float_as_uint(fmaf(__uint_as_float(v[4 * e + 2]), scale, bv.z));
+        v[4 * e + 3] = __float_as_uint(fmaf(__uint_as_float(v[4 * e + 3]), scale, bv.w));
+    }
+}
+__device__ __forceinline__ void win_pack_relu32(const uint32_t (&v)[32], int4 (&w)[4]) {
+#pragma unroll
+    for (int e = 0; e < 4; ++e) {
+        w[e].x = (int)pack_bf16x2_relu(__uint_as_float(v[8 * e]), __uint_as_float(v[8 * e + 1]));
+        w[e].y = (int)pack_bf16x2_relu(__uint_as_float(v[8 * e + 2]), __uint_as_float(v[8 * e + 3]));
+        w[e].z = (int)pack_bf16x2_relu(__uint_as_float(v[8 * e + 4]), __uint_as_float(v[8 * e + 5]));
+        w[e].w = (int)pack_bf16x2_relu(__uint_as_float(v[8 * e + 6]), __uint_as_float(v[8 * e + 7]));
+    }
 }
 
 constexpr int kConvWinThreads = 576;
@@ -210,15 +231,7 @@
                 }
                 if (!valid || g * 32 >= p.N) continue;
                 if (p.bias) {
-                    const float4* bp = reinterpret_cast<const float4*>(p.bias + g * 32);
-#pragma unroll
-                    for (int e = 0; e < 8; ++e) {
-                        const float4 bv = __ldg(bp + e);
-                        v[4 * e] = __float_as_uint(fmaf(__uint_as_float(v[4 * e]), p.scale, bv.x));
-                        v[4 * e + 1] = __float_as_uint(fmaf(__uint_as_float(v[4 * e + 1]), p.scale, bv.y));
-                        v[4 * e + 2] = __float_as_uint(fmaf(__uint_as_float(v[4 * e + 2]), p.scale, bv.z));
-                        v[4 * e + 3] = __float_as_uint(fmaf(__uint_as_float(v[4 * e + 3]), p.scale, bv.w));
-                    }
+                    win_scale_bias32(v, p.bias + g * 32, p.scale);
                 } else {
 #pragma unroll
                     for (int e = 0; e < 32; ++e) v[e] = __float_as_uint(__uint_as_float(v[e]) * p.scale);
@@ -246,13 +259,7 @@
                         w[e].w = (int)pack_f16x2_sat(__uint_as_float(v[8 * e + 6]), __uint_as_float(v[8 * e + 7]));
                     }
                 } else if (p.relu) {
-#pragma unroll
-                    for (int e = 0; e < 4; ++e) {
-                        w[e].x = (int)pack_bf16x2_relu(__uint_as_float(v[8 * e]), __uint_as_float(v[8 * e + 1]));
-                        w[e].y = (int)pack_bf16x2_relu(__uint_as_float(v[8 * e + 2]), __uint_as_float(v[8 * e + 3]));
-                        w[e].z = (int)pack_bf16x2_relu(__uint_as_float(v[8 * e + 4]), __uint_as_float(v[8 * e + 5]));
-                        w[e].w = (int)pack_bf16x2_relu(__uint_as_float(v[8 * e + 6]), __uint_as_float(v[8 * e + 7]));
-                    }
+                    win_pack_relu32(v, w);
                 } else {
 #pragma unroll
                 for (int e = 0; e < 4; ++e) {
diff --git a/cleanrl_b200/csrc/tc_heads.cuh b/cleanrl_b200/csrc/tc_heads.cuh
--- a/cleanrl_b200/csrc/tc_heads.cuh
+++ b/cleanrl_b200/csrc/tc_heads.cuh
@@ -1,6 +1,7 @@
 #pragma once
 #include "tc_base.cuh"
 #include "tc_reduce.cuh"
+#include "categorical.cuh"
 
 namespace b200rl {
 using namespace tc;
@@ -14,6 +15,36 @@
     return rpb;
 }
 
+__device__ __forceinline__ float heads_row(const bf16* __restrict__ hp, const float* sW, const float* __restrict__ bh, int A1, int lane) {
+    float hv[16];
+#pragma unroll
+    for (int q = 0; q < 2; ++q) {
+        const int4 v = ldg16(hp + q * 256 + lane * 8);
+        const uint32_t w[4] = {(uint32_t)v.x, (uint32_t)v.y, (uint32_t)v.z, (uint32_t)v.w};
+#pragma unroll
+        for (int e = 0; e < 4; ++e) {
+            hv[q * 8 + 2 * e] = __uint_as_float(w[e] << 16);
+            hv[q * 8 + 2 * e + 1] = __uint_as_float(w[e] & 0xFFFF0000u);
+        }
+    }
+    float mine = 0.f;
+    for (int a = 0; a < A1; ++a) {
+        float s = 0.f;
+#pragma unroll
+        for (int q = 0; q < 2; ++q) {
+            const float4 w0 = *reinterpret_cast<const float4*>(sW + a * 512 + q * 256 + lane * 8);
+            const float4 w1 = *reinterpret_cast<const float4*>(sW + a * 512 + q * 256 + lane * 8 + 4);
+            s = fmaf(hv[q * 8 + 0], w0.x, s); s = fmaf(hv[q * 8 + 1], w0.y, s);
+            s = fmaf(hv[q * 8 + 2], w0.z, s); s = fmaf(hv[q * 8 + 3], w0.w, s);
+            s = fmaf(hv[q * 8 + 4], w1.x, s); s = fmaf(hv[q * 8 + 5], w1.y, s);
+            s = fmaf(hv[q * 8 + 6], w1.z, s); s = fmaf(hv[q * 8 + 7], w1.w, s);
+        }
+        s = warp_sum(s);
+        if (lane == a) mine = s + bh[a];
+    }
+    return mine;
+}
+
 __global__ void __launch_bounds__(256) tc_heads_fwd(const bf16* __restrict__ hid, const float* __restrict__ Wh,
                                                     const float* __restrict__ bh, int64_t n, int A1, int H,
                                                     float* __restrict__ out) {
@@ -22,34 +53,33 @@
     __syncthreads();
     const int lane = threadIdx.x & 31, wpb = blockDim.x >> 5;
     for (int64_t row = (int64_t)blockIdx.x * wpb + (threadIdx.x >> 5); row < n; row += (int64_t)gridDim.x * wpb) {
-        float hv[16];
-        const bf16* hp = hid + row * 512;
-#pragma unroll
-        for (int q = 0; q < 2; ++q) {
-            const int4 v = ldg16(hp + q * 256 + lane * 8);
-            const uint32_t w[4] = {(uint32_t)v.x, (uint32_t)v.y, (uint32_t)v.z, (uint32_t)v.w};
-#pragma unroll
-            for (int e = 0; e < 4; ++e) {
-                hv[q * 8 + 2 * e] = __uint_as_float(w[e] << 16);
-                hv[q * 8 + 2 * e + 1] = __uint_as_float(w[e] & 0xFFFF0000u);
-            }
+        const float mine = heads_row(hid + row * 512, sW, bh, A1, lane);
+        if (lane < A1) out[row * A1 + lane] = mine;
+    }
+}
+__global__ void __launch_bounds__(256) tc_heads_sample(const bf16* __restrict__ hid, const float* __restrict__ Wh,
+                                                       const float* __restrict__ bh, int64_t n, int A,
+                                                       const float* __restrict__ noise, int64_t* __restrict__ action,
+                                                       float* __restrict__ logprob, float* __restrict__ value) {
+    extern __shared__ float sW[];
+    __shared__ float sX[8][kMaxHeads];
+    const int A1 = A + 1;
+    for (int i = threadIdx.x; i < A1 * 512; i += blockDim.x) sW[i] = Wh[i];
+    __syncthreads();
+    const int lane = threadIdx.x & 31, wid = threadIdx.x >> 5, wpb = blockDim.x >> 5;
+    float* x = sX[wid];
+    for (int64_t row = (int64_t)blockIdx.x * wpb + wid; row < n; row += (int64_t)gridDim.x * wpb) {
+        const float mine = heads_row(hid + row * 512, sW, bh, A1, lane);
+        if (lane < A1) x[lane] = mine;
+        __syncwarp();
+        if (lane == 0) {
+            const RowStats rs = row_stats(x, A);
+            const int arg = categorical_draw<false>(x, noise + row * (int64_t)A, A, rs, nullptr);
+            action[row] = arg;
+            logprob[row] = x[arg] - rs.lse;
+            value[row] = x[A];
         }
-        float mine = 0.f;
-        for (int a = 0; a < A1; ++a) {
-            float s = 0.f;
-#pragma unroll
-            for (int q = 0; q < 2; ++q) {
-                const float4 w0 = *reinterpret_cast<const float4*>(sW + a * 512 + q * 256 + lane * 8);
-                const float4 w1 = *reinterpret_cast<const float4*>(sW + a * 512 + q * 256 + lane * 8 + 4);
-                s = fmaf(hv[q * 8 + 0], w0.x, s); s = fmaf(hv[q * 8 + 1], w0.y, s);
-                s = fmaf(hv[q * 8 + 2], w0.z, s); s = fmaf(hv[q * 8 + 3], w0.w, s);
-                s = fmaf(hv[q * 8 + 4], w1.x, s); s = fmaf(hv[q * 8 + 5], w1.y, s);
-                s = fmaf(hv[q * 8 + 6], w1.z, s); s = fmaf(hv[q * 8 + 7], w1.w, s);
-            }
-            s = warp_sum(s);
-            if (lane == a) mine = s + bh[a];
-        }
-        if (lane < A1) out[row * A1 + lane] = mine;
+        __syncwarp();
     }
 }
 __global__ void __launch_bounds__(256) tc_heads_bwd_data(const float* __restrict__ dhead, const float* __restrict__ Wh,
diff --git a/cleanrl_b200/csrc/tc_rollout_tower.cuh b/cleanrl_b200/csrc/tc_rollout_tower.cuh
--- /dev/null
+++ b/cleanrl_b200/csrc/tc_rollout_tower.cuh
@@ -0,0 +1,384 @@
+#pragma once
+#include "tc_base.cuh"
+#include "tc_conv_win.cuh"
+#include "tc_conv1_u8.cuh"
+
+namespace b200rl {
+using namespace tc;
+
+struct TowerParams {
+    const uint8_t* frames;
+    uint8_t* slot_rm;
+    uint8_t* slot_cm;
+    int n;
+    const int8_t* limbs;
+    const float* sc;
+    const float* b1;
+    const bf16* w2;
+    const float* b2;
+    const bf16* w3;
+    const float* b3;
+    bf16* act3;
+};
+
+constexpr int kTwFrameRows = 224, kTwAct1Rows = 104, kTwAct2Rows = 88;
+constexpr int kTwFrame = 0;
+constexpr int kTwAct1 = kTwFrame + kTwFrameRows * 128;
+constexpr int kTwAct1Img = kTwAct1Rows * 128;
+constexpr int kTwAct2 = kTwAct1 + 2 * kTwAct1Img;
+constexpr int kTwW1 = kTwAct2 + kTwAct2Rows * 128;
+constexpr int kTwW2 = kTwW1 + 4 * 4096;
+constexpr int kTwW3 = kTwW2 + 8 * 8192;
+constexpr int kTwSmemBytes = kTwW3 + 9 * 8192;
+constexpr size_t kTwSmemAlloc = (size_t)kTwSmemBytes + 1024;
+static_assert(kTwAct1 % 1024 == 0 && kTwAct1Img % 1024 == 0 && kTwAct2 % 1024 == 0 && kTwW1 % 1024 == 0 && kTwW2 % 1024 == 0 &&
+              kTwW3 % 1024 == 0, "operand images must be 1024-byte aligned");
+static_assert(266 * 128 + 128 <= kTwAct1 + kTwAct1Img, "conv1 overrun must stay inside act1");
+static_assert(kTwAct1 + kTwAct1Img + 139 * 128 <= kTwAct2 + kTwAct2Rows * 128, "conv2 overrun must stay inside act2");
+static_assert(kTwAct2 + 148 * 128 <= kTwW2, "conv3 overrun must stay inside the conv1 limbs");
+static_assert(kTwSmemAlloc <= 227 * 1024, "tower exceeds the 227 KB of shared memory per block");
+constexpr int kTwThreads = 18 * 32;
+constexpr uint32_t kTwTmemCols = 512, kTwAcc2 = 256, kTwAcc3 = 320;
+
+template <bool RAW>
+__global__ void __launch_bounds__(kTwThreads, 1) tc_rollout_tower(const __grid_constant__ CUtensorMap tmF, const TowerParams p) {
+    extern __shared__ uint8_t smem_raw[];
+    __shared__ uint64_t fr_full, fr_empty, acc1_full, acc1_empty, a1_full, a1_empty, acc2_full, acc2_empty, a2_full, a2_empty,
+        acc3_full, acc3_empty;
+    __shared__ uint32_t tmem_base_smem;
+    __shared__ __align__(16) float s_sc[32], s_bias[32];
+    uint8_t* smem = reinterpret_cast<uint8_t*>((reinterpret_cast<uintptr_t>(smem_raw) + 1023) & ~uintptr_t(1023));
+    uint8_t* sFrame = smem + kTwFrame;
+    uint8_t* sAct1 = smem + kTwAct1;
+    uint8_t* sAct2 = smem + kTwAct2;
+    const int tid = threadIdx.x, warp = tid >> 5, lane = tid & 31;
+
+    if (tid == 0) {
+        mbar_init(&fr_full, 1); mbar_init(&fr_empty, 1);
+        mbar_init(&acc1_full, 1); mbar_init(&acc1_empty, 8);
+        mbar_init(&a1_full, 8); mbar_init(&a1_empty, 1);
+        mbar_init(&acc2_full, 1); mbar_init(&acc2_empty, 4);
+        mbar_init(&a2_full, 4); mbar_init(&a2_empty, 1);
+        mbar_init(&acc3_full, 1); mbar_init(&acc3_empty, 4);
+        fence_barrier_init();
+        if (!RAW) tma_prefetch_desc(&tmF);
+    }
+    if (warp == 1) tmem_alloc(&tmem_base_smem, kTwTmemCols);
+    {
+        constexpr int kC1 = 4 * 64 * 4, kC2 = 8 * 64 * 8, kC3 = 9 * 64 * 8, kAll = kC1 + kC2 + kC3, kBatch = 8;
+        for (int base = 0; base < kAll; base += kBatch * kTwThreads) {
+            int4 v[kBatch];
+            uint32_t dst[kBatch];
+#pragma unroll
+            for (int u = 0; u < kBatch; ++u) {
+                const int idx = base + u * kTwThreads + tid;
+                dst[u] = 0xFFFFFFFFu;
+                if (idx < kC1) {
+                    const int c16 = idx & 3, t = (idx >> 2) & 3, r = idx >> 4;
+                    dst[u] = kTwW1 + t * 4096 + img64_off(r, c16);
+                    v[u] = ldg16(p.limbs + r * 256 + t * 64 + c16 * 16);
+                } else if (idx < kC1 + kC2) {
+                    const int i = idx - kC1, c16 = i & 7, t = i >> 3, r = t % 64, j = t / 64;
+                    dst[u] = kTwW2 + j * 8192 + img_off(r, c16);
+                    v[u] = ldg16(p.w2 + (int64_t)r * 512 + j * 64 + c16 * 8);
+                } else if (idx < kAll) {
+                    const int i = idx - kC1 - kC2, c16 = i & 7, t = i >> 3, r = t % 64, j = t / 64;
+                    dst[u] = kTwW3 + j * 8192 + img_off(r, c16);
+                    v[u] = ldg16(p.w3 + (int64_t)r * 576 + j * 64 + c16 * 8);
+                }
+            }
+#pragma unroll
+            for (int u = 0; u < kBatch; ++u)
+                if (dst[u] != 0xFFFFFFFFu) *reinterpret_cast<int4*>(smem + dst[u]) = v[u];
+        }
+    }
+    if (RAW)
+        for (int idx = tid; idx < 4 * 8; idx += blockDim.x) {
+            const int r = 220 + (idx >> 3), c16 = idx & 7;
+            if (r > 220 || c16 >= 4) *reinterpret_cast<int4*>(sFrame + img_off(r, c16)) = make_int4(0, 0, 0, 0);
+        }
+    if (tid < 32) { s_sc[tid] = p.sc[32 + tid]; s_bias[tid] = p.b1[tid]; }
+    fence_proxy_async_smem();
+    tc_fence_before_sync();
+    __syncthreads();
+    tc_fence_after_sync();
+    const uint32_t tmem = tmem_base_smem;
+    const int img0 = (int)(((int64_t)p.n * blockIdx.x) / gridDim.x);
+    const int cnt = (int)(((int64_t)p.n * (blockIdx.x + 1)) / gridDim.x) - img0;
+
+    if (warp == 1) {
+        const bool leader = elect_one();
+        constexpr uint32_t idesc = make_idesc_i8(128, 64);
+        const uint64_t a_hi = desc_kmajor(0) & 0xFFFFFFFF00000000ull;
+        const uint32_t a_flags = (uint32_t)(desc_kmajor(0) & 0xFFFFFFFFull);
+        const uint64_t b_hi = desc_kmajor_sw64(0) & 0xFFFFFFFF00000000ull;
+        const uint32_t b_flags = (uint32_t)(desc_kmajor_sw64(0) & 0xFFFFFFFFull);
+        const uint32_t w_lo = ((smem_u32(smem + kTwW1) & 0x3FFFFu) >> 4) | b_flags;
+        constexpr int off[4] = {0, 1, 21, 22};
+        for (int k = 0; k < cnt; ++k) {
+            mbar_wait(&fr_full, k & 1);
+            if (k > 0) mbar_wait(&acc1_empty, (k - 1) & 1);
+            tc_fence_after_sync();
+            if (leader) {
+#pragma unroll
+                for (int tp = 0; tp < 2; ++tp) {
+                    const uint32_t win_lo = ((smem_u32(sFrame + tp * 128 * 128) & 0x3FFFFu) >> 4) | a_flags;
+#pragma unroll
+                    for (int e = 0; e < 2; ++e) {
+                        const uint32_t d_addr = tmem + (uint32_t)(2 * tp + e) * 64;
+#pragma unroll
+                        for (int t = 0; t < 4; ++t) {
+                            const int po = e + off[t];
+                            const uint32_t a_lo = win_lo + (uint32_t)((po >> 1) * 8 + (po & 1) * 4);
+                            const uint32_t b_lo = w_lo + (uint32_t)((t * 4096) >> 4);
+#pragma unroll
+                            for (int kk = 0; kk < 2; ++kk)
+                                umma_i8(d_addr, a_hi | (uint64_t)(a_lo + 2 * kk), b_hi | (uint64_t)(b_lo + 2 * kk), idesc,
+                                        (t | kk) != 0 ? 1u : 0u);
+                        }
+                    }
+                }
+                umma_commit(&fr_empty);
+                umma_commit(&acc1_full);
+            }
+            __syncwarp();
+        }
+    } else if (warp == 0) {
+        const bool leader = elect_one();
+        constexpr uint32_t idesc = make_idesc(128, 64, 0, 0);
+        const uint64_t desc_hi = desc_kmajor(0) & 0xFFFFFFFF00000000ull;
+        const uint32_t flags = (uint32_t)(desc_kmajor(0) & 0xFFFFFFFFull);
+        const uint32_t a1_lo = ((smem_u32(sAct1) & 0x3FFFFu) >> 4) | flags;
+        const uint32_t a2_lo = ((smem_u32(sAct2) & 0x3FFFFu) >> 4) | flags;
+        const uint32_t w2_lo = ((smem_u32(smem + kTwW2) & 0x3FFFFu) >> 4) | flags;
+        const uint32_t w3_lo = ((smem_u32(smem + kTwW3) & 0x3FFFFu) >> 4) | flags;
+        constexpr int sh2[4] = {0, 1, 10, 11};
+        for (int k = 0; k < cnt; ++k) {
+            mbar_wait(&a1_full, k & 1);
+            if (k > 0) mbar_wait(&acc2_empty, (k - 1) & 1);
+            tc_fence_after_sync();
+            if (leader) {
+#pragma unroll
+                for (int t = 0; t < 4; ++t) {
+#pragma unroll
+                    for (int c = 0; c < 2; ++c) {
+                        const uint32_t a_lo = a1_lo + (uint32_t)((c * kTwAct1Img) >> 4) + (uint32_t)sh2[t] * 8u;
+                        const uint32_t b_lo = w2_lo + (uint32_t)(((t * 2 + c) * 8192) >> 4);
+#pragma unroll
+                        for (int kk = 0; kk < 4; ++kk)
+                            umma_bf16(tmem + kTwAcc2, desc_hi | (uint64_t)(a_lo + 2 * kk), desc_hi | (uint64_t)(b_lo + 2 * kk), idesc,
+                                      (t | c | kk) != 0 ? 1u : 0u);
+                    }
+                }
+                umma_commit(&a1_empty);
+                umma_commit(&acc2_full);
+            }
+            __syncwarp();
+            mbar_wait(&a2_full, k & 1);
+            if (k > 0) mbar_wait(&acc3_empty, (k - 1) & 1);
+            tc_fence_after_sync();
+            if (leader) {
+#pragma unroll
+                for (int t = 0; t < 9; ++t) {
+                    const uint32_t a_lo = a2_lo + (uint32_t)((t / 3) * 9 + (t % 3)) * 8u;
+                    const uint32_t b_lo = w3_lo + (uint32_t)((t * 8192) >> 4);
+#pragma unroll
+                    for (int kk = 0; kk < 4; ++kk)
+                        umma_bf16(tmem + kTwAcc3, desc_hi | (uint64_t)(a_lo + 2 * kk), desc_hi | (uint64_t)(b_lo + 2 * kk), idesc,
+                                  (t | kk) != 0 ? 1u : 0u);
+                }
+                umma_commit(&a2_empty);
+                umma_commit(&acc3_full);
+            }
+            __syncwarp();
+        }
+    } else if (warp < 10) {
+        const int ew = warp & 3, tp = (warp - 2) >> 2;
+        const int lrow = ew * 32 + lane;
+        const uint32_t lane_base = tmem + ((uint32_t)(ew * 32) << 16);
+        for (int k = 0; k < cnt; ++k) {
+            mbar_wait(&acc1_full, k & 1);
+            if (k > 0) mbar_wait(&a1_empty, (k - 1) & 1);
+            tc_fence_after_sync();
+#pragma unroll 1
+            for (int e = 0; e < 2; ++e) {
+                uint32_t a1[32], a2[32];
+                const uint32_t lane_addr = lane_base + (uint32_t)(2 * tp + e) * 64;
+                tmem_ld32(lane_addr, a1);
+                tmem_ld32(lane_addr + 32, a2);
+                tmem_ld_wait();
+                if (e == 1) {
+                    tc_fence_before_sync();
+                    __syncwarp();
+                    if (lane == 0) mbar_arrive(&acc1_empty);
+                }
+                const int rem = 2 * ((tp << 7) + lrow) + e;
+                const int Y = (rem * 3121) >> 16, X = rem - Y * 21;
+                if (rem < 441 && Y < 20 && X < 20) {
+                    uint32_t pk[16];
+                    conv1_i8_epilogue(a1, a2, s_sc, s_bias, pk);
+                    const int cell = (Y >> 1) * 10 + (X >> 1), cls = (Y & 1) * 2 + (X & 1);
+                    uint8_t* row = sAct1 + (cls >> 1) * kTwAct1Img;
+#pragma unroll
+                    for (int j = 0; j < 4; ++j)
+                        *reinterpret_cast<int4*>(row + img_off(cell, (cls & 1) * 4 + j)) =
+                            make_int4((int)pk[4 * j], (int)pk[4 * j + 1], (int)pk[4 * j + 2], (int)pk[4 * j + 3]);
+                }
+            }
+            fence_proxy_async_smem();
+            __syncwarp();
+            if (lane == 0) mbar_arrive(&a1_full);
+        }
+    } else if (warp < 14) {
+        const int ew = warp & 3;
+        const int m = ew * 32 + lane;
+        const uint32_t lane_addr = tmem + ((uint32_t)(ew * 32) << 16);
+        const int Y2 = m / 10, X2 = m - Y2 * 10;
+        const bool v2 = m < 100 && Y2 < 9 && X2 < 9;
+        const int Y3 = m / 9, X3 = m - Y3 * 9;
+        const bool v3 = m < 81 && Y3 < 7 && X3 < 7;
+        for (int k = 0; k < cnt; ++k) {
+            mbar_wait(&acc2_full, k & 1);
+            if (k > 0) mbar_wait(&a2_empty, (k - 1) & 1);
+            tc_fence_after_sync();
+#pragma unroll 1
+            for (int g = 0; g < 2; ++g) {
+                uint32_t v[32];
+                tmem_ld32(lane_addr + kTwAcc2 + g * 32, v);
+                tmem_ld_wait();
+                if (g == 1) {
+                    tc_fence_before_sync();
+                    __syncwarp();
+                    if (lane == 0) mbar_arrive(&acc2_empty);
+                }
+                if (!v2) continue;
+                win_scale_bias32(v, p.b2 + g * 32, 1.0f);
+                int4 w[4];
+                win_pack_relu32(v, w);
+                const int r = Y2 * 9 + X2;
+#pragma unroll
+                for (int j = 0; j < 4; ++j) *reinterpret_cast<int4*>(sAct2 + img_off(r, g * 4 + j)) = w[j];
+            }
+            fence_proxy_async_smem();
+            __syncwarp();
+            if (lane == 0) mbar_arrive(&a2_full);
+            mbar_wait(&acc3_full, k & 1);
+            tc_fence_after_sync();
+            const int64_t img = img0 + k;
+#pragma unroll 1
+            for (int g = 0; g < 2; ++g) {
+                uint32_t v[32];
+                tmem_ld32(lane_addr + kTwAcc3 + g * 32, v);
+                tmem_ld_wait();
+                if (g == 1) {
+                    tc_fence_before_sync();
+                    __syncwarp();
+                    if (lane == 0) mbar_arrive(&acc3_empty);
+                }
+                if (!v3) continue;
+                win_scale_bias32(v, p.b3 + g * 32, 1.0f);
+                int4 w[4];
+                win_pack_relu32(v, w);
+                bf16* dst = p.act3 + ((img * 7 + Y3) * 7 + X3) * 64 + g * 32;
+                st_global_256(dst, w[0], w[1]);
+                st_global_256(dst + 16, w[2], w[3]);
+            }
+        }
+    } else if (RAW) {
+        const int ct = tid - 14 * 32;
+        constexpr int kItems = 112 * 4, kPer = kItems / 128 + 1;
+        for (int k = 0; k < cnt; ++k) {
+            const int64_t img = img0 + k;
+            const uint8_t* src = p.frames + img * 28224;
+            uint32_t W[kPer][16];
+#pragma unroll
+            for (int j = 0; j < kPer; ++j) {
+                const int it = ct + 128 * j;
+                const int c = it & 3, q4 = it >> 2;
+#pragma unroll
+                for (int e = 0; e < 4; ++e) {
+                    const int pos = q4 * 4 + e;
+                    const int Y = (pos * 3121) >> 16, X = pos - Y * 21;
+                    const bool ok = it < kItems && pos < 441;
+                    const uint32_t* w = reinterpret_cast<const uint32_t*>(src + c * 7056 + (Y * 4) * 84 + X * 4);
+#pragma unroll
+                    for (int sy = 0; sy < 4; ++sy) W[j][e * 4 + sy] = ok ? __ldg(w + sy * 21) : 0u;
+                }
+            }
+#pragma unroll
+            for (int j = 0; j < kPer; ++j) {
+                const int it = ct + 128 * j;
+                if (it >= kItems) continue;
+                const int c = it & 3, q4 = it >> 2;
+                uint32_t* cm = reinterpret_cast<uint32_t*>(p.slot_cm + (img * 64 + c * 16) * 448) + q4;
+#pragma unroll
+                for (int sy = 0; sy < 4; ++sy) {
+                    const uint32_t lo = prmt(W[j][sy], W[j][4 + sy], 0x5140u), hi = prmt(W[j][8 + sy], W[j][12 + sy], 0x5140u);
+                    const uint32_t lo2 = prmt(W[j][sy], W[j][4 + sy], 0x7362u), hi2 = prmt(W[j][8 + sy], W[j][12 + sy], 0x7362u);
+                    cm[(sy * 4 + 0) * 112] = prmt(lo, hi, 0x5410u);
+                    cm[(sy * 4 + 1) * 112] = prmt(lo, hi, 0x7632u);
+                    cm[(sy * 4 + 2) * 112] = prmt(lo2, hi2, 0x5410u);
+                    cm[(sy * 4 + 3) * 112] = prmt(lo2, hi2, 0x7632u);
+                }
+#pragma unroll
+                for (int e = 0; e < 4; ++e) {
+                    const int pos = q4 * 4 + e;
+                    if (pos >= 441) continue;
+                    *reinterpret_cast<int4*>(p.slot_rm + (img * 441 + pos) * 64 + c * 16) =
+                        make_int4((int)W[j][e * 4], (int)W[j][e * 4 + 1], (int)W[j][e * 4 + 2], (int)W[j][e * 4 + 3]);
+                }
+            }
+            if (k > 0) mbar_wait(&fr_empty, (k - 1) & 1);
+#pragma unroll
+            for (int j = 0; j < kPer; ++j) {
+                const int it = ct + 128 * j;
+                if (it >= kItems) continue;
+                const int c = it & 3, q4 = it >> 2;
+#pragma unroll
+                for (int e = 0; e < 4; ++e) {
+                    const int pos = q4 * 4 + e;
+                    if (pos >= 441) continue;
+                    const int q = pos >> 1;
+                    *reinterpret_cast<int4*>(sFrame + img_off(q, (pos & 1) * 4 + c)) =
+                        make_int4((int)W[j][e * 4], (int)W[j][e * 4 + 1], (int)W[j][e * 4 + 2], (int)W[j][e * 4 + 3]);
+                }
+            }
+            fence_proxy_async_smem();
+            asm volatile("bar.sync 1, 128;" ::: "memory");
+            if (ct == 0) mbar_arrive(&fr_full);
+        }
+    } else if (warp == 14) {
+        if (lane == 0) {
+            for (int k = 0; k < cnt; ++k) {
+                if (k > 0) mbar_wait(&fr_empty, (k - 1) & 1);
+                mbar_arrive_expect_tx(&fr_full, (uint32_t)(kTwFrameRows * 128));
+                tma_load_3d(smem_u32(sFrame), &tmF, 0, 0, img0 + k, &fr_full);
+            }
+        }
+        __syncwarp();
+    }
+    tc_fence_before_sync();
+    __syncthreads();
+    if (warp == 1) tmem_dealloc(tmem, kTwTmemCols);
+}
+
+static int launch_rollout_tower(const TowerParams& p, cudaStream_t s, const char* what) {
+    int grid = num_sms();
+    if (grid > p.n) grid = p.n;
+    CUtensorMap tmF;
+    memset(&tmF, 0, sizeof(tmF));
+    int rc;
+    if (p.frames) {
+        static SmemAttrCache attr;
+        if ((rc = attr.ensure(tc_rollout_tower<true>, kTwSmemAlloc, what))) return rc;
+        tc_rollout_tower<true><<<grid, kTwThreads, kTwSmemAlloc, s>>>(tmF, p);
+    } else {
+        if ((rc = make_tmap_pairs_u8(&tmF, p.slot_rm, p.n, what, kTwFrameRows))) return rc;
+        static SmemAttrCache attr;
+        if ((rc = attr.ensure(tc_rollout_tower<false>, kTwSmemAlloc, what))) return rc;
+        tc_rollout_tower<false><<<grid, kTwThreads, kTwSmemAlloc, s>>>(tmF, p);
+    }
+    return check_launch(what);
+}
+
+}
diff --git a/cleanrl_b200/ops.py b/cleanrl_b200/ops.py
--- a/cleanrl_b200/ops.py
+++ b/cleanrl_b200/ops.py
@@ -467,6 +467,29 @@
         _lib.check(rc, "naturecnn_bf16_forward")
         return head_out
 
+    def rollout_step(self, frames, slot_rm, slot_cm, flat_params, noise, action, logprob, value):
+        lib = _lib.load()
+        n = slot_rm.shape[0]
+        _contig(slot_rm, "slot_rm")
+        if tuple(slot_rm.shape[1:]) != (441, 64) or slot_rm.dtype != torch.uint8:
+            raise TypeError(f"slot_rm must be uint8 [n,441,64] (got {slot_rm.dtype} {tuple(slot_rm.shape)})")
+        if frames is not None:
+            _contig(frames, "frames"); _contig(slot_cm, "slot_cm")
+            if tuple(frames.shape) != (n, 4, 84, 84) or tuple(slot_cm.shape) != (n, 64, 448):
+                raise ValueError("frames [n,4,84,84] and slot_cm [n,64,448] must match slot_rm's n")
+        _contig(noise, "noise")
+        assert tuple(noise.shape) == (n, self.A)
+        for nm, t in (("action", action), ("logprob", logprob), ("value", value)):
+            _contig(t, nm)
+            assert t.shape[0] == n, nm
+        f = torch.float32
+        rc = lib.b200rl_naturecnn_bf16_rollout_step(
+            _ptr(frames, torch.uint8, "frames", True), _ptr(slot_rm, torch.uint8, "slot_rm"),
+            _ptr(slot_cm if frames is not None else None, torch.uint8, "slot_cm", True), n, self.A,
+            _ptr(flat_params, f, "params"), self.packed.data_ptr(), self.acts(n, 2).data_ptr(), _ptr(noise, f, "noise"),
+            _ptr(action, torch.int64, "action"), _ptr(logprob, f, "logprob"), _ptr(value, f, "value"), _stream())
+        _lib.check(rc, "naturecnn_bf16_rollout_step")
+
     def grad_tail_offset(self):
         return int(_lib.load().b200rl_naturecnn_grad_tail_offset(self.A))
 
diff --git a/cleanrl_b200/ppo_engine.py b/cleanrl_b200/ppo_engine.py
--- a/cleanrl_b200/ppo_engine.py
+++ b/cleanrl_b200/ppo_engine.py
@@ -156,16 +156,27 @@
             dst.copy_(src, non_blocking=True)
         self.h2d_bytes += src.numel() * src.element_size()
 
+    def _fused_rollout(self):
+        return self.u8_rollout and getattr(self.agent, "precision", "fp32") == "bf16" and hasattr(self.agent, "rollout_step_into")
+
+    def _rollout_step(self, step, src_u8, sl=slice(None), noise=None):
+        if self._fused_rollout():
+            self.agent.rollout_step_into(src_u8, self.obs[step][sl], self.obs_t[step][sl], self.actions[step][sl],
+                                         self.logprobs[step][sl], self.values[step][sl], noise=noise)
+            return
+        if src_u8 is not None:
+            self._to_storage(src_u8, step, sl)
+        self.agent.sample_into(self.obs[step][sl], self.actions[step][sl], self.logprobs[step][sl], self.values[step][sl],
+                               noise=noise)
+
     def _step_device_work(self, step, noise=None):
         if self.s2d:
-            self._to_storage(self.obs_u8, step)
+            return self._rollout_step(step, self.obs_u8, noise=noise)
         self.agent.sample_into(self.obs[step], self.actions[step], self.logprobs[step], self.values[step], noise=noise)
 
     def _chunk_device_work(self, step, c):
         sl = slice(*self.chunk_bounds[c])
-        self._to_storage(self.obs_u8[sl], step, sl)
-        self.agent.sample_into(self.obs[step][sl], self.actions[step][sl], self.logprobs[step][sl],
-                               self.values[step][sl], noise=self.noise_buf[sl])
+        self._rollout_step(step, self.obs_u8[sl], sl, noise=self.noise_buf[sl])
 
     def _run_step(self, step, chunk=None):
         if chunk is not None:
@@ -255,9 +266,9 @@
             for step in range(self.T):
                 src = obs_pool[step % P]
                 if self.s2d and src.dtype == torch.uint8:
-                    self._to_storage(src, step)
-                else:
-                    self.obs[step].copy_(src)
+                    self._rollout_step(step, src)
+                    continue
+                self.obs[step].copy_(src)
                 self.agent.sample_into(self.obs[step], self.actions[step], self.logprobs[step], self.values[step])
 
         if not getattr(self.agent, "graph_friendly", False):
@@ -307,7 +318,7 @@
     def _part_work(self, step, lo, hi):
         sl = slice(lo, hi)
         if self.s2d:
-            self._to_storage(self.obs_u8[sl], step, sl)
+            return self._rollout_step(step, self.obs_u8[sl], sl, noise=self._noise_bufs[step & 1][sl])
         self.agent.sample_into(self.obs[step][sl], self.actions[step][sl], self.logprobs[step][sl], self.values[step][sl],
                                noise=self._noise_bufs[step & 1][sl])
 
@@ -369,8 +380,7 @@
             ops.frames_delta_s2d_u8(self._new_d[sl], prev_rm[sl], prev_cm[sl], dst_rm[sl], dst_cm[sl],
                                     full_slot=self._slot_d[sl], full_frames=self._delta[part]["full_d"])
         if sample:
-            self.agent.sample_into(dst_rm[sl], self.actions[step][sl], self.logprobs[step][sl], self.values[step][sl],
-                                   noise=self._noise_bufs[step & 1][sl])
+            self._rollout_step(step, None, sl, noise=self._noise_bufs[step & 1][sl])
 
     @staticmethod
     def _host_pinned(arr):
diff --git a/include/b200rl.h b/include/b200rl.h
--- a/include/b200rl.h
+++ b/include/b200rl.h
@@ -157,6 +157,9 @@
 int b200rl_naturecnn_bf16_forward(const void* obs, int obs_format, const int64_t* rows, int64_t n, int A,
                                   const float* params, const void* packed, void* acts,
                                   float* head_out, void* stream);
+int b200rl_naturecnn_bf16_rollout_step(const uint8_t* frames, uint8_t* slot_rm, uint8_t* slot_cm, int64_t n, int A,
+                                       const float* params, const void* packed, void* acts, const float* noise,
+                                       int64_t* action, float* logprob, float* value, void* stream);
 int b200rl_naturecnn_bf16_backward(const void* obs, const void* obs_aux, int obs_format, const int64_t* rows, int64_t n, int A,
                                    const float* params, const void* packed, void* acts,
                                    const float* dhead, float* grads,
```
